# barlettacarmen/CrCNN

Measured on NVIDIA B200. Metric: encrypted MNIST images/sec, higher is better.
Workload: dtype u64

## Files before the change

### crcnn_b200/csrc/engine.cu

```cuda
#include <cuda_runtime.h>
#include <dlfcn.h>
#include <algorithm>
#include <cstdlib>
#include <cstring>
#include <map>
#include <unordered_map>
#include <string>
#include <vector>

#include "../../include/crcnn_b200.h"
#include "kernels.cuh"
#include "params.h"
#include "tc_mac.cuh"
#include "tcn_mac.cuh"
#include "relin32.cuh"
#include "reenc.cuh"

using namespace crcnn;

namespace {

enum KernelClass {
    KC_NTT_FWD = 0, KC_NTT_INV, KC_MAC, KC_PLAIN_EXPAND, KC_POOL, KC_BN, KC_PLAIN_OP,
    KC_BEHZ_LIFT, KC_SQ_TENSOR, KC_BEHZ_FLOOR, KC_RELIN, KC_PROBE, KC_TC_SPLIT, KC_TC_MAC, KC_TCN_SPLIT, KC_TCN_MAC, KC_RELIN32, KC_REENC, KC_COUNT
};
const char *kClassNames[KC_COUNT] = {"ntt_forward", "ntt_inverse", "weighted_sum_mac", "plain_expand_ntt", "pool_sum",
                                     "batch_norm", "plain_op", "behz_lift", "square_tensor", "behz_floor_sk",
                                     "relinearize", "imad_probe", "tc_plane_split", "weighted_sum_tc_i8", "tcn_plane_split",
                                     "weighted_sum_tcn_i8", "relinearize_u32", "reencrypt"};

thread_local std::string g_create_error;

}

struct crcnn_tensor {
    long count;
    int size;
    int ntt;
    uint64_t *d;
};

static long next_plain_serial() { static long s = 0; return ++s; }

struct crcnn_plain {
    long serial = next_plain_serial();
    long count;
    bool sparse_shape = false;
    std::vector<uint32_t> off, idx;
    std::vector<uint64_t> val;
    uint32_t *d_off = nullptr, *d_idx = nullptr;
    uint64_t *d_val = nullptr;
    uint64_t *ntt_mul = nullptr;
    uint64_t *ntt_mul_sh = nullptr;
    uint64_t *ntt_add = nullptr;
    uint64_t *coef_add = nullptr;
    int tap_state = 0;
    int tc_state = 0;
    int8_t *tc_A = nullptr;
    int tc_R = 0, tc_Kpad = 0;
    uint8_t *tcn_W = nullptr;
    int tcn_R = 0;
    bool tcn_pre = false;
    uint64_t *fused_C = nullptr, *fused_Csh = nullptr, *fused_D = nullptr;
    long fused_scale = 0, fused_mean = 0;
    int add_mult = 1;
    bool dense_only = false;
    crcnn_plain *folded_w = nullptr, *folded_b = nullptr;
    long folded_key[9] = {0, 0, 0, 0, 0, 0, 0, 0, 0};
};

struct crcnn_evk {
    uint64_t *d = nullptr;
    long key_off[MAXK];
    int digits[MAXK];
    int dbc;
    bool has_r32 = false;
    Relin32 r32;
};

struct crcnn_keys {
    uint64_t *sk = nullptr;
    uint64_t *pk = nullptr;
    ReencConsts c;
    BudgetConsts b;
};

struct crcnn_ctx {
    int device = 0;
    cudaStream_t stream = nullptr;
    HostParams hp;
    DeviceParams *dP = nullptr;
    std::vector<void *> owned;
    int n = 0, logn = 0, K = 0, S = 0;
    int chunk_terms = 1 << 30;
    size_t weight_cache_bytes = 24ull << 30;
    int sm_count = 148;
    int tc_mode = 1;
    int tc_min_fanin = 256;
    int tc_min_outputs = 32;
    int tap_mode = 1;
    int relin_mode = 1;
    int tcn_mode = 1;
    int sq_lean = 1;
    int tcn_preshift = 1;
    int tcn_fold = 1;
    size_t tc_scratch_bytes = 12ull << 30;
    std::string err;
    std::map<std::vector<int>, int *> index_cache;
    std::unordered_map<void *, size_t> big_size;
    std::multimap<size_t, void *> big_free;
    size_t big_cached = 0, big_cache_cap = 64ull << 30;
    long long st_big_malloc = 0, st_big_hit = 0, st_big_bypass = 0, st_flush = 0, st_small_malloc = 0;
    uint64_t *stage = nullptr;
    size_t stage_bytes = 0;
    bool prof_on = false;
    long launches[KC_COUNT] = {0};
    double ms[KC_COUNT] = {0};
    double work_bytes[KC_COUNT] = {0};
    double work_ops[KC_COUNT] = {0};
    struct Pending { int cls; cudaEvent_t a, b; };
    std::vector<Pending> pending;
    std::vector<cudaEvent_t> event_pool;
};

namespace {

int fail(crcnn_ctx *ctx, int code, const std::string &msg) {
    if (ctx) ctx->err = msg; else g_create_error = msg;
    return code;
}

#define CU(call)                                                                                       \
    do {                                                                                               \
        cudaError_t e__ = (call);                                                                      \
        if (e__ != cudaSuccess) {                                                                      \
            int code__ = (e__ == cudaErrorMemoryAllocation) ? CRCNN_ERR_OUT_OF_MEMORY : CRCNN_ERR_CUDA; \
            return fail(ctx, code__, std::string(#call) + ": " + cudaGetErrorString(e__));            \
        }                                                                                              \
    } while (0)

#define REQUIRE(cond, msg) \
    do { if (!(cond)) return fail(ctx, CRCNN_ERR_INVALID_ARGUMENT, msg); } while (0)

struct ProfScope {
    crcnn_ctx *c; int cls; cudaEvent_t a = nullptr, b = nullptr;
    ProfScope(crcnn_ctx *ctx, int k, double bytes = 0, double ops = 0) : c(ctx), cls(k) {
        c->launches[cls]++;
        c->work_bytes[cls] += bytes;
        c->work_ops[cls] += ops;
        if (!c->prof_on) return;
        auto get = [&]() { cudaEvent_t e; if (!c->event_pool.empty()) { e = c->event_pool.back(); c->event_pool.pop_back(); } else cudaEventCreate(&e); return e; };
        a = get(); b = get();
        cudaEventRecord(a, c->stream);
    }
    ~ProfScope() {
        if (!a) return;
        cudaEventRecord(b, c->stream);
        c->pending.push_back({cls, a, b});
    }
};

void prof_collect(crcnn_ctx *c) {
    for (auto &p : c->pending) {
        cudaEventSynchronize(p.b);
        float t = 0;
        cudaEventElapsedTime(&t, p.a, p.b);
        c->ms[p.cls] += t;
        c->event_pool.push_back(p.a);
        c->event_pool.push_back(p.b);
    }
    c->pending.clear();
}

inline size_t poly_words(const crcnn_ctx *c) { return (size_t)c->K * c->n; }
inline double lp_bytes(const crcnn_ctx *c, double polys) { return polys * c->n * 8.0; }
inline double lp_bfly(const crcnn_ctx *c, double polys) { return polys * (c->n / 2) * c->logn; }

constexpr size_t kBigBlock = 32ull << 20;
void big_cache_flush(crcnn_ctx *ctx) {
    for (auto &kv : ctx->big_free) { ctx->big_size.erase(kv.second); cudaFreeAsync(kv.second, ctx->stream); }
    ctx->big_free.clear();
    ctx->big_cached = 0;
}
int dev_alloc(crcnn_ctx *ctx, size_t bytes, void **out) {
    *out = nullptr;
    if (bytes == 0) return CRCNN_OK;
    if (bytes >= kBigBlock) {
        auto it = ctx->big_free.find(bytes);
        if (it != ctx->big_free.end()) {
            *out = it->second;
            ctx->big_cached -= bytes;
            ctx->big_free.erase(it);
            ctx->st_big_hit++;
            return CRCNN_OK;
        }
        ctx->st_big_malloc++;
    } else {
        ctx->st_small_malloc++;
    }
    cudaError_t e = cudaMallocAsync(out, bytes, ctx->stream);
    if (e == cudaErrorMemoryAllocation && !ctx->big_free.empty()) {
        cudaGetLastError();
        ctx->st_flush++;
        big_cache_flush(ctx);
        e = cudaMallocAsync(out, bytes, ctx->stream);
    }
    CU(e);
    if (bytes >= kBigBlock) ctx->big_size[*out] = bytes;
    return CRCNN_OK;
}
void dev_free(crcnn_ctx *ctx, void *p) {
    if (!p) return;
    auto it = ctx->big_size.find(p);
    if (it != ctx->big_size.end()) {
        if (ctx->big_cached + it->second <= ctx->big_cache_cap) {
            ctx->big_free.insert({it->second, p});
            ctx->big_cached += it->second;
            return;
        }
        ctx->big_size.erase(it);
        ctx->st_big_bypass++;
    }
    cudaFreeAsync(p, ctx->stream);
}

int new_tensor(crcnn_ctx *ctx, long count, int size, int ntt, crcnn_tensor **out) {
    auto *t = new crcnn_tensor{count, size, ntt, nullptr};
    int rc = dev_alloc(ctx, (size_t)count * size * poly_words(ctx) * 8, (void **)&t->d);
    if (rc) { delete t; return rc; }
    *out = t;
    return CRCNN_OK;
}

int ntt_inplace(crcnn_ctx *ctx, uint64_t *d, long npolys, int slot_base, int slot_count, bool inverse) {
    ProfScope ps(ctx, inverse ? KC_NTT_INV : KC_NTT_FWD, 2 * lp_bytes(ctx, npolys), lp_bfly(ctx, npolys));
    CU(launch_ntt(ctx->dP, ctx->logn, d, npolys, slot_base, slot_count, inverse, ctx->stream));
    return CRCNN_OK;
}

int ensure_domain(crcnn_ctx *ctx, crcnn_tensor *t, int want_ntt) {
    if (t->ntt == want_ntt) return CRCNN_OK;
    int rc = ntt_inplace(ctx, t->d, t->count * t->size * ctx->K, 0, ctx->K, !want_ntt);
    if (rc) return rc;
    t->ntt = want_ntt;
    return CRCNN_OK;
}

enum PlainForm { PF_NTT_MUL, PF_NTT_ADD, PF_COEF_ADD };

int expand_range(crcnn_ctx *ctx, crcnn_plain *p, long first, long count, PlainForm f, uint64_t *dst) {
    ProfScope ps(ctx, KC_PLAIN_EXPAND, lp_bytes(ctx, (double)count * ctx->K), f != PF_COEF_ADD ? lp_bfly(ctx, (double)count * ctx->K) : 0);
    CU(launch_plain_expand(ctx->dP, ctx->logn, ctx->K, p->d_off, p->d_idx, p->d_val, first, count,
                           (f == PF_NTT_MUL ? 0 : 1) | (p->sparse_shape ? 2 : 0), f != PF_COEF_ADD, dst, ctx->stream));
    return CRCNN_OK;
}

// ... 195 lines not shown
    dev_free(ctx, w->ntt_mul); w->ntt_mul = nullptr;
    if (w->ntt_mul_sh) { dev_free(ctx, w->ntt_mul_sh); w->ntt_mul_sh = nullptr; }
    w->tcn_R = R;
    w->tcn_pre = preshift;
    return CRCNN_OK;
}

int run_weighted_sum_tcn(crcnn_ctx *ctx, crcnn_tensor *in, crcnn_plain *w, crcnn_plain *b, const int *d_index, int R,
                         int Npos, int Pimg, int m_first, int M, crcnn_tensor *out) {
    const int Kpad = tcn_kpad(R), ncols = 2 * Npos, total = ctx->K * ctx->n;
    const int variant = ctx->tcn_mode >= 2 ? ctx->tcn_mode - 1 : 0;
    const bool want_pre = ctx->tcn_preshift && tcn_preshift_shape(R, ncols, M, variant) &&
                          7 * tcn_w_bytes(7, (int)(w->count / R), Kpad, ctx->K, ctx->n) <= ctx->weight_cache_bytes;
    int rc = ensure_domain(ctx, in, 1);
    if (!rc) rc = ensure_form(ctx, b, PF_NTT_ADD);
    if (!rc) rc = ensure_tcn_weights(ctx, w, R, want_pre);
    if (rc) return rc;
    const size_t pw = poly_words(ctx);
    const size_t per_slot = tcn_x_bytes_per_slot(7, ncols, Kpad);
    long chunk = (long)(ctx->tc_scratch_bytes / per_slot) / 32 * 32;
    chunk = std::max<long>(32, std::min<long>(chunk, total));
    uint8_t *scratch = nullptr;
    rc = dev_alloc(ctx, (size_t)chunk * per_slot, (void **)&scratch);
    if (rc) return rc;
    TcnSplitArgs s{};
    s.src = in->d; s.index = d_index; s.dst = scratch; s.item_polys = 2;
    s.R = R; s.Kpad = Kpad; s.planes = 7; s.ncols = ncols; s.n = ctx->n; s.K = ctx->K;
    TcnMacArgs a{};
    a.W = w->tcn_W; a.X = scratch; a.bias = b->ntt_add + (size_t)m_first * pw; a.out = out->d;
    a.Mall = (int)(w->count / R); a.m_first = m_first; a.M = M;
    a.R = R; a.Kpad = Kpad; a.planes = 7; a.ncols = ncols;
    a.Pimg = Pimg; a.Mtotal = M; a.m0 = 0; a.n = ctx->n; a.K = ctx->K;
    a.variant = variant;
    a.preshift = want_pre && w->tcn_pre;
    a.use_fold = ctx->tcn_fold;
    for (int j = 0; j < ctx->K; j++) a.fold[j] = tcn_fold_make(ctx->hp.d.tab[j].mod.q);
    for (long s0 = 0; s0 < total && !rc; s0 += chunk) {
        const int ns = (int)std::min<long>(chunk, total - s0);
        s.slot0 = a.slot0 = (int)s0; s.nslots = a.nslots = ns;
        const double xbytes = (double)ns * per_slot;
        cudaError_t e;
        { ProfScope ps(ctx, KC_TCN_SPLIT, (double)ncols * R * ns * 8.0 + xbytes, 0); e = launch_tcn_split(s, ctx->stream); }
        if (e == cudaSuccess) {
            ProfScope ps(ctx, KC_TCN_MAC, xbytes + (double)ns * 7 * M * Kpad * (a.preshift ? 7 : 1) + (double)ncols * M * ns * 8.0, (double)ns * ncols * M * R * 49.0);
            e = launch_tcn_mac(ctx->dP, a, ctx->sm_count, ctx->stream);
        }
        if (e != cudaSuccess) rc = fail(ctx, CRCNN_ERR_CUDA, std::string("limb-split tensor-core weighted sum: ") + cudaGetErrorString(e));
    }
    dev_free(ctx, scratch);
    if (!rc) out->ntt = 1;
    return rc;
}

int run_weighted_sum(crcnn_ctx *ctx, crcnn_tensor *in, crcnn_plain *w, crcnn_plain *b, const int *d_index, int R,
                     int Npos, int Pimg, int Mall, int m_first, int M, crcnn_tensor *out) {
    if (ctx->tc_mode && R >= ctx->tc_min_fanin && (ctx->tc_mode == 2 || Mall >= ctx->tc_min_outputs) && w->sparse_shape && tc_mac_available() == cudaSuccess) {
        int rc = ensure_tc_form(ctx, w, R);
        if (rc) return rc;
        if (w->tc_state == 1) return run_weighted_sum_tc(ctx, in, w, b, d_index, R, Npos, Pimg, m_first, M, out);
    }
    if (ctx->tcn_mode && tcn_planes_for(ctx->hp.d) == 7 && R <= TCN_MAX_R && w->count % R == 0 && tc_mac_available() == cudaSuccess &&
        (w->tcn_W || tcn_w_bytes(7, (int)(w->count / R), tcn_kpad(R), ctx->K, ctx->n) <= ctx->weight_cache_bytes))
        return run_weighted_sum_tcn(ctx, in, w, b, d_index, R, Npos, Pimg, m_first, M, out);
    int rc = ensure_domain(ctx, in, 1);
    if (rc) return rc;
    rc = ensure_form(ctx, b, PF_NTT_ADD);
    if (rc) return rc;
    MacArgs a{};
    a.x = in->d; a.in_index = d_index; a.out = out->d;
    a.R = R; a.Npos = Npos; a.Pimg = Pimg; a.Mtotal = M; a.K = ctx->K; a.n = ctx->n;
    a.chunk_terms = ctx->chunk_terms;
    const size_t pw = poly_words(ctx);
    const size_t all_bytes = (size_t)w->count * pw * 8;
    if (w->ntt_mul || all_bytes <= ctx->weight_cache_bytes) {
        rc = ensure_form(ctx, w, PF_NTT_MUL);
        if (rc) return rc;
        a.w = w->ntt_mul + (size_t)m_first * R * pw;
        a.bias = b->ntt_add + (size_t)m_first * pw;
        a.M = M; a.m0 = 0;
        ProfScope ps(ctx, KC_MAC, lp_bytes(ctx, ((double)in->count + (double)M * Npos) * 2 * ctx->K + (double)M * R * ctx->K),
                     (double)M * Npos * R * 2 * ctx->K * ctx->n);
        CU(launch_mac(ctx->dP, a, ctx->stream));
        return CRCNN_OK;
    }
    long rows = (long)std::max<size_t>(1, ctx->weight_cache_bytes / ((size_t)R * pw * 8));
    rows = std::min<long>(rows, M);
    uint64_t *scratch = nullptr;
    rc = dev_alloc(ctx, (size_t)rows * R * pw * 8, (void **)&scratch);
    if (rc) return rc;
    for (long m0 = 0; m0 < M; m0 += rows) {
        long cur = std::min<long>(rows, M - m0);
        rc = expand_range(ctx, w, (long)(m_first + m0) * R, cur * R, PF_NTT_MUL, scratch);
        if (rc) break;
        a.w = scratch; a.bias = b->ntt_add + (size_t)(m_first + m0) * pw;
        a.M = (int)cur; a.m0 = (int)m0;
        ProfScope ps(ctx, KC_MAC, lp_bytes(ctx, ((double)in->count + (double)cur * Npos) * 2 * ctx->K + (double)cur * R * ctx->K),
                     (double)cur * Npos * R * 2 * ctx->K * ctx->n);
        cudaError_t e = launch_mac(ctx->dP, a, ctx->stream);
        if (e != cudaSuccess) { rc = fail(ctx, CRCNN_ERR_CUDA, cudaGetErrorString(e)); break; }
    }
    dev_free(ctx, scratch);
    return rc;
}

int upload_rows(crcnn_ctx *ctx, const uint64_t *host, size_t rows, uint64_t *dst, cudaStream_t s) {
    const size_t n = ctx->n;
    if (rows * n * 8 < (8u << 20)) {
        CU(cudaMemcpy2DAsync(dst, n * 8, host, (n + 1) * 8, n * 8, rows, cudaMemcpyHostToDevice, s));
        return CRCNN_OK;
    }
    uint64_t *stage = nullptr;
    CU(cudaMallocAsync((void **)&stage, rows * (n + 1) * 8, s));
    cudaError_t e = cudaMemcpyAsync(stage, host, rows * (n + 1) * 8, cudaMemcpyHostToDevice, s);
    if (e == cudaSuccess) e = launch_strip_pad(stage, dst, (long)rows, (int)n, s);
    cudaFreeAsync(stage, s);
    if (e != cudaSuccess) return fail(ctx, CRCNN_ERR_CUDA, std::string("upload: ") + cudaGetErrorString(e));
    return CRCNN_OK;
}

}

extern "C" {

const char *crcnn_last_error(const crcnn_ctx *ctx) { return ctx ? ctx->err.c_str() : g_create_error.c_str(); }

int crcnn_ctx_create(int n, int K, const uint64_t *q, uint64_t t, int device, crcnn_ctx **out) {
    crcnn_ctx *ctx = nullptr;
    if (!out || !q) return fail(nullptr, CRCNN_ERR_INVALID_ARGUMENT, "null argument");
    *out = nullptr;
    int ndev = 0;
    if (cudaGetDeviceCount(&ndev) != cudaSuccess || ndev == 0)
        return fail(nullptr, CRCNN_ERR_NO_DEVICE, "no CUDA device: crcnn_b200 has no CPU fallback");
    if (device < 0 || device >= ndev) return fail(nullptr, CRCNN_ERR_INVALID_ARGUMENT, "bad device ordinal");
    HostParams hp;
    try {
        hp = derive_params(n, K, q, t);
    } catch (const std::exception &e) {
        return fail(nullptr, CRCNN_ERR_INVALID_ARGUMENT, e.what());
    }
    CU(cudaSetDevice(device));
    auto *c = new crcnn_ctx();
    c->device = device; c->n = n; c->K = K; c->S = hp.d.S; c->logn = hp.d.logn;
    int maxbits = 0;
    for (int i = 0; i < K; i++) { int b = 0; for (uint64_t v = q[i]; v; v >>= 1) b++; maxbits = std::max(maxbits, b); }
    int spare = 128 - 2 * maxbits;
    c->chunk_terms = spare >= 30 ? (1 << 30) : (1 << spare);
    cudaDeviceGetAttribute(&c->sm_count, cudaDevAttrMultiProcessorCount, device);
    if (const char *e = getenv("CRCNN_TC")) c->tc_mode = atoi(e);
    if (const char *e = getenv("CRCNN_TCN")) c->tcn_mode = atoi(e);
    if (const char *e = getenv("CRCNN_TAP")) c->tap_mode = atoi(e);
    if (const char *e = getenv("CRCNN_TCN_FOLD")) c->tcn_fold = atoi(e);
    if (const char *e = getenv("CRCNN_TCN2_PRESHIFT")) c->tcn_preshift = atoi(e);
    if (const char *e = getenv("CRCNN_SQ_LEAN")) c->sq_lean = atoi(e);
    cudaMemPool_t pool;
    if (cudaDeviceGetDefaultMemPool(&pool, device) == cudaSuccess) {
        uint64_t thr = UINT64_MAX;
        cudaMemPoolSetAttribute(pool, cudaMemPoolAttrReleaseThreshold, &thr);
    }
    {
        size_t fr = 0, tot = 0;
        if (cudaMemGetInfo(&fr, &tot) == cudaSuccess && tot) c->big_cache_cap = tot / 4 * 3;
    }
    int slots = K + hp.d.S;
    auto up = [&](const std::vector<uint64_t> &v, const uint64_t **dst) -> cudaError_t {
        void *d = nullptr;
        cudaError_t e = cudaMalloc(&d, v.size() * 8);
        if (e != cudaSuccess) return e;
        c->owned.push_back(d);
        *dst = (const uint64_t *)d;
        return cudaMemcpy(d, v.data(), v.size() * 8, cudaMemcpyHostToDevice);
    };
    cudaError_t e = cudaSuccess;
    for (int s = 0; s < slots && e == cudaSuccess; s++) {
        std::vector<uint64_t> fw(2 * (size_t)n), bw(2 * (size_t)n);
        for (int i = 0; i < n; i++) {
            fw[2 * i] = hp.w[s][i]; fw[2 * i + 1] = hp.wp[s][i];
            bw[2 * i] = hp.iwf[s][i]; bw[2 * i + 1] = hp.iwfp[s][i];
        }
        e = up(fw, &hp.d.tab[s].w);
        if (e == cudaSuccess) e = up(bw, &hp.d.tab[s].iw);
        const int NG = n >> 4;
        std::vector<uint64_t> fl(2 * (size_t)16 * NG, 0), bl(2 * (size_t)16 * NG, 0);
        for (int G = 0; G < NG; G++)
            for (int st = 0; st < 4; st++) {
                for (int lb = 0; lb < (1 << st); lb++) {
                    const size_t at = 2 * ((size_t)((1 << st) - 1 + lb) * NG + G), from = 2 * ((((size_t)NG + G) << st) + lb);
                    fl[at] = fw[from]; fl[at + 1] = fw[from + 1];
                }
                for (int lb = 0; lb < (1 << (3 - st)); lb++) {
                    const size_t at = 2 * ((size_t)(16 - (16 >> st) + lb) * NG + G);
                    const size_t from = 2 * ((size_t)((n >> 1) >> st) + ((size_t)G << (3 - st)) + lb);
                    bl[at] = bw[from]; bl[at + 1] = bw[from + 1];
                }
            }
        if (e == cudaSuccess) e = up(fl, &hp.d.tab[s].wl);
        if (e == cudaSuccess) e = up(bl, &hp.d.tab[s].iwl);
        hp.d.tab[s].tf = nullptr;
        if (e == cudaSuccess && s < K) e = up(hp.tf[s], &hp.d.tab[s].tf);
    }
    if (e == cudaSuccess) e = cudaMalloc((void **)&c->dP, sizeof(DeviceParams));
    if (e == cudaSuccess) e = cudaMemcpy(c->dP, &hp.d, sizeof(DeviceParams), cudaMemcpyHostToDevice);
    if (e != cudaSuccess) {
        std::string m = cudaGetErrorString(e);
        for (void *p : c->owned) cudaFree(p);
        if (c->dP) cudaFree(c->dP);
        delete c;
        return fail(nullptr, CRCNN_ERR_CUDA, "context setup: " + m);
    }
    c->hp = std::move(hp);
    *out = c;
    return CRCNN_OK;
}

int crcnn_ctx_destroy(crcnn_ctx *ctx) {
    if (!ctx) return CRCNN_OK;
    cudaSetDevice(ctx->device);
    big_cache_flush(ctx);
    cudaStreamSynchronize(ctx->stream);
    prof_collect(ctx);
    for (auto e : ctx->event_pool) cudaEventDestroy(e);
    for (auto &kv : ctx->index_cache) cudaFree(kv.second);
    if (ctx->stage) cudaFree(ctx->stage);
    for (void *p : ctx->owned) cudaFree(p);
    cudaFree(ctx->dP);
    delete ctx;
    return CRCNN_OK;
}

int crcnn_ctx_set_stream(crcnn_ctx *ctx, void *cuda_stream) {
    if (!ctx) return CRCNN_ERR_INVALID_ARGUMENT;
    CU(cudaStreamSynchronize(ctx->stream));
    ctx->stream = (cudaStream_t)cuda_stream;
    return CRCNN_OK;
}

int crcnn_ctx_sync(crcnn_ctx *ctx) {
    if (!ctx) return CRCNN_ERR_INVALID_ARGUMENT;
    CU(cudaStreamSynchronize(ctx->stream));
    prof_collect(ctx);
    return CRCNN_OK;
}

int crcnn_ctx_alloc_stats(crcnn_ctx *ctx, long long out[6]) {
    if (!ctx || !out) return CRCNN_ERR_INVALID_ARGUMENT;
    out[0] = ctx->st_big_malloc; out[1] = ctx->st_big_hit; out[2] = ctx->st_big_bypass; out[3] = ctx->st_flush;
    out[4] = ctx->st_small_malloc; out[5] = (long long)ctx->big_cached;
    return CRCNN_OK;
}

int crcnn_ctx_set_weight_cache_bytes(crcnn_ctx *ctx, size_t bytes) {
    if (!ctx) return CRCNN_ERR_INVALID_ARGUMENT;
    ctx->weight_cache_bytes = bytes;
    return CRCNN_OK;
}

int crcnn_ctx_set_tensor_core_mode(crcnn_ctx *ctx, int mode, int min_fanin, size_t scratch_bytes) {
    if (!ctx) return CRCNN_ERR_INVALID_ARGUMENT;
    REQUIRE(mode >= 0 && mode <= 2, "tensor-core mode must be 0, 1 or 2");
    ctx->tc_mode = mode;
    if (min_fanin > 0) ctx->tc_min_fanin = min_fanin;
    if (scratch_bytes > 0) ctx->tc_scratch_bytes = scratch_bytes;
    return CRCNN_OK;
}

int crcnn_ctx_set_limb_split_mode(crcnn_ctx *ctx, int mode) {
    if (!ctx) return CRCNN_ERR_INVALID_ARGUMENT;
    REQUIRE(mode >= 0 && mode <= 3, "limb-split mode must be 0 (off), 1 (on), 2 (row-major kernel) or 3 (column-major kernel)");
    ctx->tcn_mode = mode;
    return CRCNN_OK;
}

int crcnn_ctx_set_limb_split_reduction(crcnn_ctx *ctx, int mode) {
    if (!ctx) return CRCNN_ERR_INVALID_ARGUMENT;
    REQUIRE(mode == 0 || mode == 1, "limb-split reduction must be 0 (128-bit recombination + Barrett) or 1 (folded through 2^k - delta)");
    ctx->tcn_fold = mode;
    return CRCNN_OK;
}

int crcnn_ctx_set_relin_mode(crcnn_ctx *ctx, int mode) {
    if (!ctx) return CRCNN_ERR_INVALID_ARGUMENT;
    REQUIRE(mode == 0 || mode == 1, "relinearize mode must be 0 (64-bit transforms) or 1 (word-size auxiliary primes)");
    ctx->relin_mode = mode;
    return CRCNN_OK;
}

int crcnn_ctx_ntt_table(const crcnn_ctx *ctx_c, int slot, int which, uint64_t *out) {
    crcnn_ctx *ctx = const_cast<crcnn_ctx *>(ctx_c);
    if (!ctx) return CRCNN_ERR_INVALID_ARGUMENT;
    REQUIRE(out && slot >= 0 && slot < ctx->K + ctx->S && which >= 0 && which < 4, "bad table selector");
    const auto &v = which == 0 ? ctx->hp.w[slot] : which == 1 ? ctx->hp.wp[slot] : which == 2 ? ctx->hp.iw[slot] : ctx->hp.iwp[slot];
    memcpy(out, v.data(), v.size() * 8);
    return CRCNN_OK;
}

int crcnn_ctx_bsk_count(const crcnn_ctx *ctx) { return ctx ? ctx->S : CRCNN_ERR_INVALID_ARGUMENT; }

int crcnn_tensor_upload_ex(crcnn_ctx *ctx, const uint64_t *host, long count, int size, int ntt_form, crcnn_tensor **out) {
    if (!ctx) return CRCNN_ERR_INVALID_ARGUMENT;
    REQUIRE(host && out && count >= 0 && size >= 2 && size <= 3, "bad tensor upload arguments");
    CU(cudaSetDevice(ctx->device));
    crcnn_tensor *t = nullptr;
    int rc = new_tensor(ctx, count, size, ntt_form ? 1 : 0, &t);
    if (rc) return rc;
    const size_t n = ctx->n, rows = (size_t)count * size * ctx->K;
    if (rows) {
        int rc2 = upload_rows(ctx, host, rows, t->d, ctx->stream);
// ... 594 lines not shown
        int rc = get_index_table(ctx, key, table, &d_index);
        if (rc) return rc;
    } else {
        d_index = ctx->index_cache[key];
    }
    int rc = ensure_pool_bn_consts(ctx, scale, mean, invstd);
    if (rc) return rc;
    crcnn_tensor *o = nullptr;
    rc = new_tensor(ctx, Nout, 2, 1, &o);
    if (rc) return rc;
    {
        ProfScope ps(ctx, KC_POOL, lp_bytes(ctx, ((double)in->count + Nout) * 2 * ctx->K), (double)Nout * (R + 1) * 2 * ctx->K * ctx->n);
        cudaError_t e = launch_pool(ctx->dP, ctx->n, ctx->K, in->d, d_index, Nout, R, invstd->fused_C, invstd->fused_Csh, true, o->d, ctx->stream,
                                    xo * yo, zd, invstd->fused_D);
        if (e != cudaSuccess) { crcnn_tensor_free(ctx, o); return fail(ctx, CRCNN_ERR_CUDA, cudaGetErrorString(e)); }
    }
    *out = o;
    return CRCNN_OK;
}

int crcnn_conv_pool_bn_forward_shard(crcnn_ctx *ctx, crcnn_tensor *in, crcnn_plain *w, crcnn_plain *b, int batch, int xd, int yd, int zd,
                                     int xs, int ys, int xf, int yf, int nf, int pxs, int pys, int pxf, int pyf, crcnn_plain *scale,
                                     crcnn_plain *mean, crcnn_plain *invstd, int k0, int kc, crcnn_tensor **out) {
    if (!ctx) return CRCNN_ERR_INVALID_ARGUMENT;
    REQUIRE(k0 >= 0 && kc >= 0 && k0 + kc <= nf, "bad output-channel shard");
    REQUIRE(in && w && b && mean && invstd && out, "null argument");
    REQUIRE(batch > 0 && xd > 0 && yd > 0 && zd > 0 && xs > 0 && ys > 0 && xf > 0 && yf > 0 && nf > 0 && xf <= xd && yf <= yd,
            "bad convolution geometry");
    const int cxo = (xd - xf) / xs + 1, cyo = (yd - yf) / ys + 1;
    REQUIRE(pxs > 0 && pys > 0 && pxf > 0 && pyf > 0 && pxf <= cxo && pyf <= cyo, "bad pooling geometry");
    const int pxo = (cxo - pxf) / pxs + 1, pyo = (cyo - pyf) / pys + 1;
    const int Rp = pxf * pyf, R = zd * xf * yf;
    REQUIRE(in->size == 2 && in->count == (long)batch * zd * xd * yd, "input tensor does not match the layer geometry");
    REQUIRE(w->count == (long)nf * R && b->count == nf, "kernel/bias count does not match the layer geometry");
    REQUIRE((!scale || scale->count >= 1) && mean->count == nf && invstd->count == nf, "mean/var count does not match the channel count");
    CU(cudaSetDevice(ctx->device));
    const bool pooled_grid = pxs <= pxf && pys <= pyf && xs <= xf && ys <= yf && pxs * xs <= xf && pys * ys <= yf && Rp <= 64 && sum_fits_64(ctx, Rp) &&
                             ctx->tcn_mode && tcn_planes_for(ctx->hp.d) == 7 && R <= TCN_MAX_R && tc_mac_available() == cudaSuccess &&
                             tcn_w_bytes(7, nf, tcn_kpad(R), ctx->K, ctx->n) <= ctx->weight_cache_bytes && !getenv("CRCNN_NO_POOLED_CONV");
    if (!pooled_grid) {
        if (k0 != 0 || kc != nf)
            return fail(ctx, CRCNN_ERR_UNSUPPORTED, "channel shards of conv + pool + batch-norm need the pooled-grid path");
        crcnn_tensor *mid = nullptr;
        int rc = crcnn_conv_forward(ctx, in, w, b, batch, xd, yd, zd, xs, ys, xf, yf, nf, &mid);
        if (rc) return rc;
        rc = crcnn_pool_bn_forward(ctx, mid, batch, cxo, cyo, nf, pxs, pys, pxf, pyf, scale, mean, invstd, out);
        crcnn_tensor_free(ctx, mid);
        return rc;
    }
    int rc = ensure_pool_bn_consts(ctx, scale, mean, invstd);
    if (rc) return rc;
    const long key[9] = {b->serial, scale ? scale->serial : -1, mean->serial, invstd->serial, (long)Rp, 0, 0, 0, 0};
    if (!w->folded_w || memcmp(key, w->folded_key, sizeof(key)) != 0) {
        if (w->folded_w) { crcnn_plain_free(ctx, w->folded_w); w->folded_w = nullptr; }
        if (w->folded_b) { crcnn_plain_free(ctx, w->folded_b); w->folded_b = nullptr; }
        const size_t pw = poly_words(ctx);
        rc = make_plain(ctx, std::vector<uint32_t>(w->off), std::vector<uint32_t>(w->idx), std::vector<uint64_t>(w->val), &w->folded_w);
        if (rc) return rc;
        w->folded_w->sparse_shape = false;
        w->folded_w->tc_state = -1; w->folded_w->tap_state = -1;
        rc = ensure_form(ctx, w->folded_w, PF_NTT_MUL);
        if (rc) return rc;
        CU(launch_fold_affine(ctx->dP, w->folded_w->ntt_mul, (long)nf * R, (long)pw, R, invstd->fused_C, nullptr, ctx->stream));
        rc = make_plain(ctx, std::vector<uint32_t>(b->off), std::vector<uint32_t>(b->idx), std::vector<uint64_t>(b->val), &w->folded_b);
        if (rc) return rc;
        w->folded_b->add_mult = Rp;
        rc = ensure_form(ctx, w->folded_b, PF_NTT_ADD);
        if (rc) return rc;
        CU(launch_fold_affine(ctx->dP, w->folded_b->ntt_add, (long)nf, (long)pw, 1, invstd->fused_C, invstd->fused_D, ctx->stream));
        memcpy(w->folded_key, key, sizeof(key));
    }
    const int sxd = xd - (pxf - 1) * xs, syd = yd - (pyf - 1) * ys;
    const int Nsum = batch * zd * sxd * syd;
    std::vector<int> skey = {4, batch, xd, yd, zd, xs, ys, pxf, pyf};
    const int *d_index = nullptr;
    if (ctx->index_cache.find(skey) == ctx->index_cache.end()) {
        std::vector<int> table((size_t)Nsum * Rp);
        size_t o = 0;
        for (int bz = 0; bz < batch * zd; bz++)
            for (int u = 0; u < sxd; u++)
                for (int v = 0; v < syd; v++)
                    for (int a = 0; a < pxf; a++)
                        for (int c = 0; c < pyf; c++) table[o++] = (bz * xd + u + a * xs) * yd + v + c * ys;
        rc = get_index_table(ctx, skey, table, &d_index);
        if (rc) return rc;
    } else {
        d_index = ctx->index_cache[skey];
    }
    crcnn_tensor *sums = nullptr, *pooled = nullptr;
    rc = new_tensor(ctx, Nsum, 2, in->ntt, &sums);
    if (rc) return rc;
    {
        ProfScope ps(ctx, KC_POOL, lp_bytes(ctx, ((double)in->count + Nsum) * 2 * ctx->K), (double)Nsum * Rp * 2 * ctx->K * ctx->n);
        cudaError_t e = launch_pool(ctx->dP, ctx->n, ctx->K, in->d, d_index, Nsum, Rp, nullptr, nullptr, true, sums->d, ctx->stream);
        if (e != cudaSuccess) { crcnn_tensor_free(ctx, sums); return fail(ctx, CRCNN_ERR_CUDA, cudaGetErrorString(e)); }
    }
    rc = crcnn_conv_forward_shard(ctx, sums, w->folded_w, w->folded_b, batch, sxd, syd, zd, pxs * xs, pys * ys, xf, yf, nf, k0, kc, &pooled);
    crcnn_tensor_free(ctx, sums);
    if (rc) return rc;
    if (pooled->count != (long)batch * kc * pxo * pyo || !pooled->ntt) {
        crcnn_tensor_free(ctx, pooled);
        return fail(ctx, CRCNN_ERR_UNSUPPORTED, "pooled-grid convolution produced an unexpected shape");
    }
    *out = pooled;
    return CRCNN_OK;
}

int crcnn_conv_pool_bn_forward(crcnn_ctx *ctx, crcnn_tensor *in, crcnn_plain *w, crcnn_plain *b, int batch, int xd, int yd, int zd,
                               int xs, int ys, int xf, int yf, int nf, int pxs, int pys, int pxf, int pyf, crcnn_plain *scale,
                               crcnn_plain *mean, crcnn_plain *invstd, crcnn_tensor **out) {
    return crcnn_conv_pool_bn_forward_shard(ctx, in, w, b, batch, xd, yd, zd, xs, ys, xf, yf, nf, pxs, pys, pxf, pyf, scale, mean, invstd, 0, nf, out);
}

int crcnn_bn_forward(crcnn_ctx *ctx, crcnn_tensor *in, int batch, int zd, int xd, int yd, crcnn_plain *mean,
                     crcnn_plain *invstd, crcnn_tensor **out) {
    if (!ctx) return CRCNN_ERR_INVALID_ARGUMENT;
    REQUIRE(in && mean && invstd && out, "null argument");
    REQUIRE(batch > 0 && zd > 0 && xd > 0 && yd > 0, "bad batch-norm geometry");
    REQUIRE(in->size == 2 && in->count == (long)batch * zd * xd * yd, "input tensor does not match the layer geometry");
    REQUIRE(mean->count == zd && invstd->count == zd, "mean/var count does not match the channel count");
    CU(cudaSetDevice(ctx->device));
    if (!in->ntt && ctx->tap_mode && tap_eligible(ctx, invstd)) {
        int rc = ensure_form(ctx, mean, PF_COEF_ADD);
        if (rc) return rc;
        crcnn_tensor *o = nullptr;
        rc = new_tensor(ctx, in->count, 2, 0, &o);
        if (rc) return rc;
        TapMulArgs a{};
        a.in = in->d; a.in_index = nullptr; a.R = 1; a.sub = mean->coef_add;
        a.t_off = invstd->d_off; a.t_idx = invstd->d_idx; a.t_val = invstd->d_val; a.per_channel = xd * yd; a.channels = zd;
        a.out = o->d; a.nout = in->count;
        ProfScope ps(ctx, KC_BN, lp_bytes(ctx, (double)in->count * 4 * ctx->K), (double)in->count * 2 * ctx->K * ctx->n);
        cudaError_t e = launch_tapmul(ctx->dP, ctx->n, ctx->K, a, ctx->stream);
        if (e != cudaSuccess) { crcnn_tensor_free(ctx, o); return fail(ctx, CRCNN_ERR_CUDA, cudaGetErrorString(e)); }
        *out = o;
        return CRCNN_OK;
    }
    int rc = ensure_domain(ctx, in, 1);
    if (!rc) rc = ensure_form(ctx, mean, PF_NTT_ADD);
    if (!rc) rc = ensure_shoup(ctx, invstd);
    if (rc) return rc;
    crcnn_tensor *o = nullptr;
    rc = new_tensor(ctx, in->count, 2, 1, &o);
    if (rc) return rc;
    {
        ProfScope ps(ctx, KC_BN, lp_bytes(ctx, (double)in->count * 4 * ctx->K), (double)in->count * 2 * ctx->K * ctx->n);
        cudaError_t e = launch_bn(ctx->dP, ctx->n, ctx->K, in->d, in->count, xd * yd, zd, mean->ntt_add, invstd->ntt_mul, invstd->ntt_mul_sh, o->d, ctx->stream);
        if (e != cudaSuccess) { crcnn_tensor_free(ctx, o); return fail(ctx, CRCNN_ERR_CUDA, cudaGetErrorString(e)); }
    }
    *out = o;
    return CRCNN_OK;
}

int crcnn_square(crcnn_ctx *ctx, crcnn_tensor *in, crcnn_tensor **out3) {
    if (!ctx) return CRCNN_ERR_INVALID_ARGUMENT;
    REQUIRE(in && out3, "null argument");
    REQUIRE(in->size == 2, "square expects size-2 ciphertexts");
    CU(cudaSetDevice(ctx->device));
    const bool have_ntt = in->ntt != 0;
    const bool lean = ctx->sq_lean != 0, fold = lean && behz_fold_ok(ctx->hp.d), copy_ninv = !(lean && have_ntt);
    crcnn_tensor *o = nullptr;
    int rc = new_tensor(ctx, in->count, 3, 0, &o);
    if (rc) return rc;
    const int KS = ctx->K + ctx->S;
    const size_t n = ctx->n, pw = poly_words(ctx);
    const long step = std::max<long>(1, std::min<long>(in->count, (long)((2ull << 30) / (5 * (size_t)KS * n * 8))));
    uint64_t *ext = nullptr, *prod = nullptr, *coef = nullptr;
    rc = dev_alloc(ctx, (size_t)step * 2 * KS * n * 8, (void **)&ext);
    if (!rc) rc = dev_alloc(ctx, (size_t)step * 3 * KS * n * 8, (void **)&prod);
    if (!rc && have_ntt) rc = dev_alloc(ctx, (size_t)step * 2 * pw * 8, (void **)&coef);
    if (rc) { crcnn_tensor_free(ctx, o); return rc; }
    for (long c0 = 0; c0 < in->count && !rc; c0 += step) {
        const long cur = std::min<long>(step, in->count - c0);
        const uint64_t *src = in->d + c0 * 2 * pw;
        cudaError_t e = cudaSuccess;
        if (have_ntt) {
            ProfScope ps(ctx, KC_NTT_INV, 2 * lp_bytes(ctx, (double)cur * 2 * ctx->K), lp_bfly(ctx, (double)cur * 2 * ctx->K));
            e = launch_ntt_grouped(ctx->dP, ctx->logn, coef, cur * 2 * ctx->K, 0, ctx->K, true, ctx->K, 0, ctx->stream, src,
                                   nullptr, 1, 1, copy_ninv);
        }
        if (e == cudaSuccess) { ProfScope ps(ctx, KC_BEHZ_LIFT, lp_bytes(ctx, (double)cur * 2 * (ctx->K + (have_ntt ? ctx->S : KS))), (double)cur * 2 * n * ctx->S * (ctx->K + 1)); e = launch_behz_lift(ctx->hp.d, ctx->n, have_ntt ? coef : src, have_ntt ? src : nullptr, cur, ext, ctx->stream, copy_ninv); }
        if (e == cudaSuccess) {
            if (have_ntt) {
                ProfScope ps(ctx, KC_NTT_FWD, 2 * lp_bytes(ctx, (double)cur * 2 * ctx->S), lp_bfly(ctx, (double)cur * 2 * ctx->S));
                e = launch_ntt_grouped(ctx->dP, ctx->logn, ext, cur * 2 * ctx->S, ctx->K, ctx->S, false, KS, ctx->K, ctx->stream);
            } else {
                ProfScope ps(ctx, KC_NTT_FWD, 2 * lp_bytes(ctx, (double)cur * 2 * KS), lp_bfly(ctx, (double)cur * 2 * KS));
                e = launch_ntt(ctx->dP, ctx->logn, ext, cur * 2 * KS, 0, KS, false, ctx->stream);
            }
        }
        if (e == cudaSuccess) {
            ProfScope ps(ctx, KC_SQ_TENSOR, lp_bytes(ctx, (double)cur * 5 * KS), lp_bfly(ctx, (double)cur * 3 * KS));
            e = launch_ntt_inv_tensor(ctx->dP, ctx->logn, ext, have_ntt ? src : nullptr, cur, KS, prod, fold, !lean, ctx->stream);
        }
        if (e == cudaSuccess) { ProfScope ps(ctx, KC_BEHZ_FLOOR, lp_bytes(ctx, (double)cur * 3 * (KS + ctx->K)),
                                                     (double)cur * 3 * n * (ctx->S * (ctx->K + 1) + ctx->S + ctx->K * ctx->S)); e = launch_behz_floor(ctx->hp.d, ctx->n, prod, cur, o->d + c0 * 3 * pw, ctx->stream, !lean); }
        if (e != cudaSuccess) rc = fail(ctx, CRCNN_ERR_CUDA, cudaGetErrorString(e));
    }
    dev_free(ctx, coef);
    dev_free(ctx, ext); dev_free(ctx, prod);
    if (rc) { crcnn_tensor_free(ctx, o); return rc; }
    *out3 = o;
    return CRCNN_OK;
}

int crcnn_relinearize(crcnn_ctx *ctx, crcnn_tensor *in3, crcnn_evk *evk, crcnn_tensor **out2) {
    if (!ctx) return CRCNN_ERR_INVALID_ARGUMENT;
    REQUIRE(in3 && evk && out2, "null argument");
    REQUIRE(in3->size == 3, "relinearize expects size-3 ciphertexts");
    int total_digits = 0;
    for (int i = 0; i < ctx->K; i++) {
        int bits = 0; for (uint64_t v = ctx->hp.d.tab[i].mod.q; v; v >>= 1) bits++;
        REQUIRE(evk->digits[i] * evk->dbc >= bits, "not enough evaluation keys");
        total_digits += evk->digits[i];
    }
    REQUIRE(total_digits <= 63, "too many key digits for 128-bit lazy accumulation");
    CU(cudaSetDevice(ctx->device));
    int rc = ensure_domain(ctx, in3, 0);
    if (rc) return rc;
    crcnn_tensor *o = nullptr;
    rc = new_tensor(ctx, in3->count, 2, 0, &o);
    if (rc) return rc;
    const size_t pw = poly_words(ctx);
    if (evk->has_r32 && ctx->relin_mode == 1) {
        const Relin32Consts &c = evk->r32.c;
        const size_t per_ct = relin32_scratch_bytes(ctx->n, ctx->K, c);
        const long step = std::max<long>(1, std::min<long>(std::min<long>(in3->count, 200000), (long)((2ull << 30) / per_ct)));
        void *scratch = nullptr;
        rc = dev_alloc(ctx, (size_t)step * per_ct, &scratch);
        if (rc) { crcnn_tensor_free(ctx, o); return rc; }
        for (long c0 = 0; c0 < in3->count && !rc; c0 += step) {
            const long cnt = std::min<long>(step, in3->count - c0);
            ProfScope ps(ctx, KC_RELIN32, lp_bytes(ctx, (double)cnt * 5 * ctx->K),
                         lp_bfly(ctx, (double)cnt * (c.D + 2 * ctx->K) * c.S3));
            cudaError_t e = relin32_run(ctx->dP, ctx->logn, ctx->K, evk->r32, in3->d + c0 * 3 * pw, o->d + c0 * 2 * pw, cnt, scratch, ctx->stream);
            if (e != cudaSuccess) rc = fail(ctx, CRCNN_ERR_CUDA, cudaGetErrorString(e));
        }
        dev_free(ctx, scratch);
        if (rc) { crcnn_tensor_free(ctx, o); return rc; }
        *out2 = o;
        return CRCNN_OK;
    }
    RelinArgs a{};
    a.evk = evk->d; a.dbc = evk->dbc;
    for (int i = 0; i < MAXK; i++) { a.key_off[i] = evk->key_off[i]; a.digits[i] = evk->digits[i]; }
    const size_t per_ct = (size_t)(1 + total_digits + 2) * pw * 8;
    const long step = std::max<long>(1, std::min<long>(in3->count, (long)((2ull << 30) / per_ct)));
    uint64_t *scratch = nullptr;
    rc = dev_alloc(ctx, (size_t)step * per_ct, (void **)&scratch);
    if (rc) { crcnn_tensor_free(ctx, o); return rc; }
    a.dsc = scratch;
    a.dig = scratch + (size_t)step * pw;
    a.acc = a.dig + (size_t)step * total_digits * pw;
    for (long c0 = 0; c0 < in3->count && !rc; c0 += step) {
        a.count = std::min<long>(step, in3->count - c0);
        a.in3 = in3->d + c0 * 3 * pw;
        a.out = o->d + c0 * 2 * pw;
        cudaError_t e;
        { ProfScope ps(ctx, KC_RELIN, lp_bytes(ctx, (double)a.count * 3 * ctx->K), lp_bfly(ctx, (double)a.count * total_digits * ctx->K)); e = launch_relin(ctx->dP, ctx->logn, ctx->K, a, ctx->stream); }
        if (e == cudaSuccess) {
            ProfScope ps(ctx, KC_NTT_INV, 2 * lp_bytes(ctx, (double)a.count * 2 * ctx->K) + lp_bytes(ctx, (double)a.count * 2 * ctx->K), lp_bfly(ctx, (double)a.count * 2 * ctx->K));
            e = launch_ntt_grouped(ctx->dP, ctx->logn, a.out, a.count * 2 * ctx->K, 0, ctx->K, true, ctx->K, 0, ctx->stream, a.acc, a.in3,
                                   2 * ctx->K, 3 * ctx->K);
        }
        if (e != cudaSuccess) rc = fail(ctx, CRCNN_ERR_CUDA, cudaGetErrorString(e));
    }
    dev_free(ctx, scratch);
    if (rc) { crcnn_tensor_free(ctx, o); return rc; }
    *out2 = o;
    return CRCNN_OK;
}

int crcnn_square_forward(crcnn_ctx *ctx, crcnn_tensor *in, crcnn_evk *evk, crcnn_tensor **out) {
    if (!ctx) return CRCNN_ERR_INVALID_ARGUMENT;
    crcnn_tensor *t3 = nullptr;
    int rc = crcnn_square(ctx, in, &t3);
    if (rc) return rc;
    rc = crcnn_relinearize(ctx, t3, evk, out);
    crcnn_tensor_free(ctx, t3);
    return rc;
}

int crcnn_transform_to_ntt(crcnn_ctx *ctx, crcnn_tensor *t) {
    if (!ctx) return CRCNN_ERR_INVALID_ARGUMENT;
    REQUIRE(t, "null argument");
    REQUIRE(!t->ntt, "tensor is already in NTT form");
    CU(cudaSetDevice(ctx->device));
    return ensure_domain(ctx, t, 1);
}
int crcnn_transform_from_ntt(crcnn_ctx *ctx, crcnn_tensor *t) {
    if (!ctx) return CRCNN_ERR_INVALID_ARGUMENT;
    REQUIRE(t, "null argument");
    REQUIRE(t->ntt, "tensor is not in NTT form");
    CU(cudaSetDevice(ctx->device));
    return ensure_domain(ctx, t, 0);
}

int crcnn_plain_op(crcnn_ctx *ctx, crcnn_tensor *t, crcnn_plain *p, long index, int op) {
    if (!ctx) return CRCNN_ERR_INVALID_ARGUMENT;
    REQUIRE(t && p && index >= 0 && index < p->count && op >= 0 && op <= 2, "bad plain_op arguments");
    CU(cudaSetDevice(ctx->device));
    int rc;
    const uint64_t *pl, *pl_sh = nullptr;
    if (op == 0) {
        rc = ensure_domain(ctx, t, 1);
        if (!rc) rc = ensure_shoup(ctx, p);
        if (rc) return rc;
        pl = p->ntt_mul + index * poly_words(ctx);
        pl_sh = p->ntt_mul_sh + index * poly_words(ctx);
    } else {
        rc = ensure_form(ctx, p, t->ntt ? PF_NTT_ADD : PF_COEF_ADD);
        if (rc) return rc;
        pl = (t->ntt ? p->ntt_add : p->coef_add) + index * poly_words(ctx);
    }
    ProfScope ps(ctx, KC_PLAIN_OP, lp_bytes(ctx, (double)t->count * (op == 0 ? t->size : 1) * 2 * ctx->K), (double)t->count * (op == 0 ? t->size : 1) * ctx->K * ctx->n);
    CU(launch_plain_op(ctx->dP, ctx->n, ctx->K, t->d, t->count, t->size, pl, pl_sh, op, ctx->stream));
    return CRCNN_OK;
}

int crcnn_add_many(crcnn_ctx *ctx, crcnn_tensor *t, crcnn_tensor **out) {
    if (!ctx) return CRCNN_ERR_INVALID_ARGUMENT;
    REQUIRE(t && out, "null argument");
    REQUIRE(t->count >= 1, "encrypteds cannot be empty");
    REQUIRE(t->size == 2, "add_many is implemented for size-2 ciphertexts");
    CU(cudaSetDevice(ctx->device));
    auto pass = [&](const uint64_t *src, long first, int nout, int g, uint64_t *dst) -> int {
        std::vector<int> key = {4, (int)first, nout, g};
        const int *d_index = nullptr;
        auto it = ctx->index_cache.find(key);
        if (it == ctx->index_cache.end()) {
            std::vector<int> table((size_t)nout * g);
            for (size_t i = 0; i < table.size(); i++) table[i] = (int)(first + (long)i);
            int rc = get_index_table(ctx, key, table, &d_index);
            if (rc) return rc;
        } else d_index = it->second;
        ProfScope ps(ctx, KC_POOL, lp_bytes(ctx, ((double)nout * g + nout) * 2 * ctx->K), (double)nout * g * 2 * ctx->K * ctx->n);
        CU(launch_pool(ctx->dP, ctx->n, ctx->K, src, d_index, nout, g, nullptr, nullptr, sum_fits_64(ctx, g), dst, ctx->stream));
        return CRCNN_OK;
    };
    crcnn_tensor *o = nullptr;
    int rc = new_tensor(ctx, 1, 2, t->ntt, &o);
    if (rc) return rc;
    if (t->count <= 128) {
        rc = pass(t->d, 0, 1, (int)t->count, o->d);
    } else {
        int g = 1;
        while ((long)g * g < t->count) g++;
        const long full = t->count / g, tail = t->count % g, groups = full + (tail ? 1 : 0);
        crcnn_tensor *part = nullptr;
        rc = new_tensor(ctx, groups, 2, t->ntt, &part);
        if (!rc) rc = pass(t->d, 0, (int)full, g, part->d);
        if (!rc && tail) rc = pass(t->d, full * g, 1, (int)tail, part->d + full * 2 * poly_words(ctx));
        if (!rc) rc = pass(part->d, 0, 1, (int)groups, o->d);
        crcnn_tensor_free(ctx, part);
    }
    if (rc) { crcnn_tensor_free(ctx, o); return rc; }
    *out = o;
    return CRCNN_OK;
}

int crcnn_prof_enable(crcnn_ctx *ctx, int on) {
    if (!ctx) return CRCNN_ERR_INVALID_ARGUMENT;
    ctx->prof_on = on != 0;
    return CRCNN_OK;
}
int crcnn_prof_reset(crcnn_ctx *ctx) {
    if (!ctx) return CRCNN_ERR_INVALID_ARGUMENT;
    prof_collect(ctx);
    for (int i = 0; i < KC_COUNT; i++) { ctx->launches[i] = 0; ctx->ms[i] = 0; ctx->work_bytes[i] = 0; ctx->work_ops[i] = 0; }
    return CRCNN_OK;
}
int crcnn_prof_count(crcnn_ctx *ctx) { return ctx ? (int)KC_COUNT : (int)CRCNN_ERR_INVALID_ARGUMENT; }
int crcnn_prof_get(crcnn_ctx *ctx, int cls, char *name, long *launches, double *ms) {
    if (!ctx) return CRCNN_ERR_INVALID_ARGUMENT;
    REQUIRE(cls >= 0 && cls < KC_COUNT, "bad kernel class");
    prof_collect(ctx);
    if (name) { strncpy(name, kClassNames[cls], 31); name[31] = 0; }
    if (launches) *launches = ctx->launches[cls];
    if (ms) *ms = ctx->ms[cls];
    return CRCNN_OK;
}

int crcnn_prof_get_work(crcnn_ctx *ctx, int cls, double *bytes, double *ops) {
    if (!ctx) return CRCNN_ERR_INVALID_ARGUMENT;
    REQUIRE(cls >= 0 && cls < KC_COUNT, "bad kernel class");
    if (bytes) *bytes = ctx->work_bytes[cls];
    if (ops) *ops = ctx->work_ops[cls];
    return CRCNN_OK;
}

int crcnn_probe_pipe(crcnn_ctx *ctx, int which, int blocks, int threads, int iters, double *ms, double *ops) {
    if (!ctx) return CRCNN_ERR_INVALID_ARGUMENT;
    REQUIRE(which >= 0 && which <= 4 && blocks > 0 && threads > 0 && threads <= 1024 && iters > 0 && ms, "bad probe arguments");
    CU(cudaSetDevice(ctx->device));
    uint64_t *sink = nullptr;
    int rc = dev_alloc(ctx, 8, (void **)&sink);
    if (rc) return rc;
    cudaEvent_t a, b;
    CU(cudaEventCreate(&a));
    CU(cudaEventCreate(&b));
    ctx->launches[KC_PROBE]++;
    double work = 0;
    CU(cudaEventRecord(a, ctx->stream));
    if (which == 0) { CU(launch_imad_probe(blocks, threads, iters, sink, ctx->stream)); work = (double)blocks * threads * iters * 8.0; }
    else if (which == 1) { CU(launch_imad_wide_probe(blocks, threads, iters, sink, ctx->stream)); work = (double)blocks * threads * iters * 16.0; }
    else CU(launch_umma_i8_probe(blocks, iters, which - 2, &work, ctx->stream));
    CU(cudaEventRecord(b, ctx->stream));
    CU(cudaEventSynchronize(b));
    float t = 0;
    cudaEventElapsedTime(&t, a, b);
    *ms = t;
    if (ops) *ops = work;
    cudaEventDestroy(a); cudaEventDestroy(b);
    dev_free(ctx, sink);
    return CRCNN_OK;
}
int crcnn_probe_imad(crcnn_ctx *ctx, int blocks, int threads, int iters, double *ms) {
    return crcnn_probe_pipe(ctx, 0, blocks, threads, iters, ms, nullptr);
}

int crcnn_pinned_alloc(size_t bytes, void **out) {
    if (!out) return CRCNN_ERR_INVALID_ARGUMENT;
    *out = nullptr;
    cudaError_t e = cudaHostAlloc(out, bytes, cudaHostAllocDefault);
    if (e != cudaSuccess) { g_create_error = std::string("cudaHostAlloc: ") + cudaGetErrorString(e); return e == cudaErrorMemoryAllocation ? CRCNN_ERR_OUT_OF_MEMORY : CRCNN_ERR_CUDA; }
    return CRCNN_OK;
}
int crcnn_pinned_free(void *p) { return (!p || cudaFreeHost(p) == cudaSuccess) ? CRCNN_OK : CRCNN_ERR_CUDA; }

int crcnn_stream_create(crcnn_ctx *ctx, void **stream) {
    if (!ctx) return CRCNN_ERR_INVALID_ARGUMENT;
    REQUIRE(stream, "null argument");
    CU(cudaSetDevice(ctx->device));
// ... 363 lines not shown
```

### crcnn_b200/csrc/host_selftest.cpp

```cpp
#include <cinttypes>
#include <cstdio>
#include <cstdlib>
#include <vector>
#include "params.h"

using namespace crcnn;

static uint64_t fnv(const std::vector<uint64_t> &v) {
    uint64_t h = 1469598103934665603ULL;
    for (uint64_t x : v) { h ^= x; h *= 1099511628211ULL; }
    return h;
}

int main(int argc, char **argv) {
    if (argc < 4) { fprintf(stderr, "usage: host_selftest n t q...\n"); return 2; }
    int n = atoi(argv[1]);
    uint64_t t = strtoull(argv[2], nullptr, 0);
    std::vector<uint64_t> q;
    for (int i = 3; i < argc; i++) q.push_back(strtoull(argv[i], nullptr, 0));
    try {
        HostParams hp = derive_params(n, (int)q.size(), q.data(), t);
        const DeviceParams &d = hp.d;
        printf("K %d L %d S %d half %" PRIu64 "\n", d.K, d.L, d.S, d.half);
        for (int s = 0; s < d.K + d.S; s++) {
            printf("slot %d q %" PRIu64 " r0 %" PRIu64 " r1 %" PRIu64 " root %" PRIu64 " w %" PRIu64 " wp %" PRIu64 " iw %" PRIu64 " iwp %" PRIu64 "\n",
                   s, d.tab[s].mod.q, d.tab[s].mod.r0, d.tab[s].mod.r1, hp.roots[s], fnv(hp.w[s]), fnv(hp.wp[s]), fnv(hp.iw[s]), fnv(hp.iwp[s]));
        }
        for (int j = 0; j < d.K; j++)
            printf("prime %d delta %" PRIu64 " rho %" PRIu64 " lift %" PRIu64 "\n", j, d.delta[j], d.rho[j], d.lift_inc[j]);
        uint64_t x = 0x123456789abcdef1ULL, y = 0xfedcba9876543211ULL;
        for (int s = 0; s < d.K + d.S; s++) {
            const Mod &m = d.tab[s].mod;
            for (int it = 0; it < 1000; it++) {
                x = x * 6364136223846793005ULL + 1442695040888963407ULL;
                y = y * 2862933555777941757ULL + 3037000493ULL;
                uint64_t a = x % (4 * m.q), b = y % m.q;
                uint64_t want = (uint64_t)(((unsigned __int128)a * b) % m.q);
                if (mulmod(a, b, m) != want) { printf("MULMOD MISMATCH\n"); return 1; }
                uint64_t wp = (uint64_t)((((unsigned __int128)b) << 64) / m.q);
                uint64_t lazy = mulshoup_lazy(a, b, wp, m.q);
                if (lazy >= 2 * m.q || lazy % m.q != want) { printf("SHOUP MISMATCH\n"); return 1; }
            }
        }
        for (int j = 0; j < d.K; j++) {
            const Mod &m = d.tab[j].mod;
            const TcnFold f = tcn_fold_make(m.q);
            printf("fold %d ok %u T %u delta %u\n", j, f.ok, f.T, f.delta);
            if (!f.ok) continue;
            for (int it = 0; it < 200000; it++) {
                uint32_t s[13];
                const int mode = it % 8;
                for (int w = 0; w < 13; w++) {
                    x = x * 6364136223846793005ULL + 1442695040888963407ULL;
                    const uint32_t r = (uint32_t)(x >> 33);
                    s[w] = mode == 0 ? 0x7fffffffu : mode == 1 ? 0u : mode == 2 ? ((x >> 20) & 1 ? 0x7fffffffu : 0u)
                         : mode == 3 ? 7u * 4096u * 255u * 255u - (r & 3) : mode == 4 ? (r >> (x & 31)) : r;
                }
                y = y * 2862933555777941757ULL + 3037000493ULL;
                const uint64_t bias = mode == 0 ? m.q - 1 : (it & 1) ? y % m.q : 0;
                unsigned __int128 z = 0;
                for (int w = 12; w >= 0; w--) z = (z << 8) + s[w];
                const uint64_t want = (uint64_t)((z + bias) % m.q);
                if (tcn_fold_reduce(s, bias, f, m.q) != want) { printf("FOLD MISMATCH\n"); return 1; }
            }
        }
        for (int j = 0; j < d.K; j++) {
            const Mod &m = d.tab[j].mod;
            const TcnFold f = tcn_fold_make(m.q);
            long checked = 0;
            for (int it = 0; it < 20000; it++) {
                x = x * 6364136223846793005ULL + 1442695040888963407ULL;
                y = y * 2862933555777941757ULL + 3037000493ULL;
                const uint64_t W = it < 2 ? m.q - 1 : x % m.q, X = it < 2 ? m.q - 1 : y % m.q;
                uint32_t C[7] = {0, 0, 0, 0, 0, 0, 0};
                for (int b = 0; b < 7; b++) {
                    const uint64_t wb = (uint64_t)(((unsigned __int128)1 << (8 * b)) % m.q);
                    const uint64_t wbp = (uint64_t)(((unsigned __int128)wb << 64) / m.q);
                    uint64_t Wb = mulshoup_lazy(W, wb, wbp, m.q);
                    Wb = Wb >= m.q ? Wb - m.q : Wb;
                    if (Wb != (uint64_t)(((unsigned __int128)W << (8 * b)) % m.q)) { printf("PRESHIFT MISMATCH\n"); return 1; }
                    uint64_t back = 0;
                    for (int a = 6; a >= 0; a--) back = (back << 8) | ((Wb >> (8 * a)) & 0xff);
                    if (back != Wb) { printf("PLANE MISMATCH\n"); return 1; }
                    for (int a = 0; a < 7; a++) C[a] += (uint32_t)(((X >> (8 * b)) & 0xff) * ((Wb >> (8 * a)) & 0xff));
                }
                const uint64_t bias = (it & 1) ? y % m.q : 0;
                const uint64_t want = (uint64_t)(((unsigned __int128)W * X + bias) % m.q);
                const U128 z = tcn7_combine(C);
                if (addmod(barrett128(z, m), bias, m.q) != want) { printf("SEVEN-CLASS MISMATCH\n"); return 1; }
                if (f.ok7 && tcn7_fold_reduce(C, bias, f, m.q) != want) { printf("FOLD7 MISMATCH\n"); return 1; }
                checked++;
            }
            const uint32_t cmax = 7u * 4096u * 255u * 255u;
            for (int it = 0; it < 2000 && f.ok7; it++) {
                uint32_t C[7];
                x = x * 6364136223846793005ULL + 1442695040888963407ULL;
                for (int a = 0; a < 7; a++) C[a] = it == 0 ? cmax : cmax - (uint32_t)((x >> (4 * a)) % 4096);
                const uint64_t bias = it == 0 ? m.q - 1 : x % m.q;
                unsigned __int128 z = 0;
                for (int a = 6; a >= 0; a--) z = (z << 8) + C[a];
                if (z >> 80) { printf("FOLD7 BOUND\n"); return 1; }
                if (tcn7_fold_reduce(C, bias, f, m.q) != (uint64_t)((z + bias) % m.q)) { printf("FOLD7 MISMATCH\n"); return 1; }
                checked++;
            }
            printf("fold7 %d ok7 %u checked %ld\n", j, f.ok7, checked);
        }
        for (int sidx = 0; sidx < d.K + d.S; sidx++) {
            const Mod &m = d.tab[sidx].mod;
            const Fold128 f = fold128_make(m.q);
            printf("fold128 %d ok %u delta %u\n", sidx, f.ok, f.delta);
            if (!f.ok) continue;
            for (int it = 0; it < 200000; it++) {
                x = x * 6364136223846793005ULL + 1442695040888963407ULL;
                y = y * 2862933555777941757ULL + 3037000493ULL;
                U128 z;
                const int mode = it % 8;
                z.lo = mode == 0 ? ~0ull : mode == 1 ? 0 : mode == 2 ? m.q - 1 : mode == 3 ? m.q : x;
                z.hi = mode == 0 ? ~0ull : mode == 1 ? 0 : mode == 2 ? 0 : mode == 3 ? (y >> (y & 63)) : mode == 4 ? (y >> 40) : y;
                const uint64_t want = (uint64_t)(((((unsigned __int128)z.hi) << 64) | z.lo) % m.q);
                if (reduce128_fold(z, f) != want || barrett128(z, m) != want) { printf("FOLD128 MISMATCH\n"); return 1; }
            }
        }
        typedef unsigned __int128 u128;
        for (int s = 0; s < d.K + d.S; s++) {
            const uint64_t q = d.tab[s].mod.q;
            const bool ok_ninv = (u128)d.tab[s].ninv * (uint64_t)n % q == 1;
            bool ok = ok_ninv;
            if (s < d.K) {
                ok = ok && d.mt_inv_qhat_n[s] < q && (u128)d.mt_inv_qhat_n[s] * (uint64_t)n % q == d.mt_inv_qhat[s];
                ok = ok && d.fl_c_n[s] < q && (u128)d.fl_c_n[s] * (uint64_t)n % q == d.fl_c[s];
            } else {
                ok = ok && d.fl_T_n[s - d.K] < q && (u128)d.fl_T_n[s - d.K] * (uint64_t)n % q == d.fl_T[s - d.K];
            }
            printf("ninv %d ok %d\n", s, ok ? 1 : 0);
            if (!ok) { printf("NINV CONSTANT MISMATCH\n"); return 1; }
        }
        for (int s = 0; s < d.K + d.S; s++) {
            const uint64_t q = d.tab[s].mod.q, nq = 0 - q;
            const uint64_t ws[] = {0, 1, q - 1, q / 2, 0x5555555555555555ULL % q, 0};
            long checked = 0;
            for (int wi = 0; wi < 6; wi++) {
                uint64_t w = ws[wi];
                for (int it = 0; it < 20000; it++) {
                    x = x * 6364136223846793005ULL + 1442695040888963407ULL;
                    y = y * 2862933555777941757ULL + 3037000493ULL;
                    if (wi == 5) w = y % q;
                    const uint64_t wp = (uint64_t)(((u128)w << 64) / q);
                    const int mode = it % 8;
                    const uint64_t yv = mode == 0 ? 0 : mode == 1 ? ~0ull : mode == 2 ? (x % (~0ull / q + 1)) * q
                                      : mode == 3 ? (~0ull / q) * q : mode == 4 ? q - 1 : mode == 5 ? 8 * q - 1 - (x & 7) : x;
                    const uint64_t r = mulshoup_lazy4(yv, w, wp, nq);
                    if (r >= 4 * q || r % q != (uint64_t)((u128)w * yv % q)) { printf("SHOUP4 MISMATCH\n"); return 1; }
                    const uint64_t a = x % q;
                    const U128 z = sqr128(a);
                    if (((u128)z.hi << 64 | z.lo) != (u128)a * a) { printf("SQR128 MISMATCH\n"); return 1; }
                    checked++;
                }
            }
            printf("shoup4 %d checked %ld\n", s, checked);
            const int k = reduce64_shape_k(q);
            if (k) {
                for (int it = 0; it < 200000; it++) {
                    x = x * 6364136223846793005ULL + 1442695040888963407ULL;
                    const int mode = it % 6;
                    const uint64_t v = mode == 0 ? ~0ull : mode == 1 ? 0 : mode == 2 ? q : mode == 3 ? q - 1 : mode == 4 ? (x % 16) * q + (x >> 60) : x;
                    if (reduce64_shape(v, q, k) != v % q || reduce64(v, d.tab[s].mod) != v % q) { printf("REDUCE64 MISMATCH\n"); return 1; }
                }
            }
            printf("reduce64_shape %d k %d\n", s, k);
        }
        for (int i = 4; i >= 0; i--) {
            double vals[] = {0.0867, -3.25, 0.0, 1.0, 2.8215};
            std::vector<uint32_t> idx; std::vector<uint64_t> val;
            encode_fractional_sparse(vals[i], n, t, idx, val);
            printf("enc %.4f nnz %zu", vals[i], idx.size());
            for (size_t e = 0; e < idx.size(); e++) printf(" %u:%" PRIu64, idx[e], val[e]);
            printf("\n");
        }
        printf("OK\n");
    } catch (const std::exception &e) {
        printf("ERROR %s\n", e.what());
        return 1;
    }
    return 0;
}
```

### crcnn_b200/csrc/kernels.cu

```cuda
#include "kernels.cuh"
#include "devcfg.cuh"
#include "ntt.cuh"
#include <cstdlib>
#include <cstring>

namespace crcnn {

template <int LOGN>
__global__ void __launch_bounds__(NttPlan<LOGN>::THREADS, NttPlan<LOGN>::MIN_CTAS)
ntt_fwd_kernel(uint64_t *__restrict__ data, const DeviceParams *__restrict__ P, int slot_base, int slot_count, int group_polys,
               int group_off) {
    extern __shared__ uint64_t sm[];
    const long p = blockIdx.x;
    const NttTable tb = P->tab[slot_base + (int)(p % slot_count)];
    uint64_t *poly = data + ((p / slot_count) * group_polys + group_off + p % slot_count) * (1L << LOGN);
    ntt_forward_to_smem<LOGN>(sm, poly, tb);
    smem_store_poly_canonical<LOGN>(sm, poly, tb.mod);
}

template <int LOGN, bool NINV>
__global__ void __launch_bounds__(NttPlan<LOGN>::THREADS, NttPlan<LOGN>::MIN_CTAS)
ntt_inv_kernel(uint64_t *__restrict__ data, const DeviceParams *__restrict__ P, int slot_base, int slot_count, int group_polys,
               int group_off, const uint64_t *__restrict__ src, const uint64_t *__restrict__ addend, int add_group, int add_stride) {
    extern __shared__ uint64_t sm[];
// ... 586 lines not shown
}

cudaError_t launch_tapmul(const DeviceParams *P, int n, int K, const TapMulArgs &a, cudaStream_t stream) {
    if (a.nout <= 0) return cudaSuccess;
    const long blocks = a.nout * 2 * K * (n / TAP_CT);
    if (n % TAP_CT || blocks > 0x7fffffffL) return cudaErrorInvalidValue;
    tapmul_kernel<<<(unsigned)blocks, 256, 0, stream>>>(P, a);
    return cudaGetLastError();
}

__global__ void __launch_bounds__(256)
shoup_companion_kernel(const DeviceParams *__restrict__ P, const uint64_t *__restrict__ data, long words, uint64_t *__restrict__ out) {
    const long w = (long)blockIdx.x * 256 + threadIdx.x;
    if (w >= words) return;
    const uint64_t q = P->tab[(w / P->n) % P->K].mod.q;
    out[w] = (uint64_t)((((unsigned __int128)__ldg(data + w)) << 64) / q);
}

cudaError_t launch_shoup_companion(const DeviceParams *P, const uint64_t *data, long words, uint64_t *out, cudaStream_t stream) {
    if (words <= 0) return cudaSuccess;
    shoup_companion_kernel<<<(unsigned)((words + 255) / 256), 256, 0, stream>>>(P, data, words, out);
    return cudaGetLastError();
}

__global__ void __launch_bounds__(256)
scale_small_kernel(const DeviceParams *__restrict__ P, uint64_t *__restrict__ data, long words, int times) {
    const long w = (long)blockIdx.x * 256 + threadIdx.x;
    if (w >= words) return;
    const uint64_t q = P->tab[(w / P->n) % P->K].mod.q;
    const uint64_t v = data[w];
    uint64_t acc = 0;
    for (int i = 0; i < times; i++) acc = addmod(acc, v, q);
    data[w] = acc;
}

__global__ void __launch_bounds__(256)
fold_affine_kernel(const DeviceParams *__restrict__ P, uint64_t *__restrict__ data, long rows, int group, const uint64_t *__restrict__ C,
                   const uint64_t *__restrict__ D) {
    const long pw = (long)P->K * P->n;
    const long w = (long)blockIdx.x * 256 + threadIdx.x;
    if (w >= rows * pw) return;
    const long row = w / pw, lw = w - row * pw;
    const Mod mod = P->tab[lw / P->n].mod;
    const long cw = (row / group) * pw + lw;
    uint64_t v = mulmod(data[w], __ldg(C + cw), mod);
    if (D) v = submod(v, __ldg(D + cw), mod.q);
    data[w] = v;
}

cudaError_t launch_fold_affine(const DeviceParams *P, uint64_t *data, long rows, long poly_words, int group, const uint64_t *C,
                               const uint64_t *D, cudaStream_t stream) {
    if (rows <= 0) return cudaSuccess;
    fold_affine_kernel<<<(unsigned)((rows * poly_words + 255) / 256), 256, 0, stream>>>(P, data, rows, group, C, D);
    return cudaGetLastError();
}

__global__ void __launch_bounds__(256)
fold_fc_input_affine_kernel(const DeviceParams *__restrict__ P, uint64_t *__restrict__ W, int out_dim, int in_dim, int per_channel,
                            const uint64_t *__restrict__ C, const uint64_t *__restrict__ D, uint64_t *__restrict__ Bias) {
    const long pw = (long)P->K * P->n;
    const long id = (long)blockIdx.x * 256 + threadIdx.x;
    if (id >= (long)out_dim * pw) return;
    const long k = id / pw, lw = id - k * pw;
    const Mod mod = P->tab[lw / P->n].mod;
    uint64_t acc = Bias[k * pw + lw];
    for (int r = 0; r < in_dim; r++) {
        const long cw = (long)(r / per_channel) * pw + lw;
        uint64_t *wp = W + ((long)k * in_dim + r) * pw + lw;
        const uint64_t w = *wp;
        acc = submod(acc, mulmod(w, __ldg(D + cw), mod), mod.q);
        *wp = mulmod(w, __ldg(C + cw), mod);
    }
    Bias[k * pw + lw] = acc;
}

cudaError_t launch_fold_fc_input_affine(const DeviceParams *P, uint64_t *W, int out_dim, int in_dim, long poly_words, int per_channel,
                                        const uint64_t *C, const uint64_t *D, uint64_t *Bias, cudaStream_t stream) {
    if (out_dim <= 0 || in_dim <= 0) return cudaSuccess;
    fold_fc_input_affine_kernel<<<(unsigned)((out_dim * poly_words + 255) / 256), 256, 0, stream>>>(P, W, out_dim, in_dim, per_channel, C, D, Bias);
    return cudaGetLastError();
}

cudaError_t launch_scale_small(const DeviceParams *P, uint64_t *data, long words, int times, cudaStream_t stream) {
    if (words <= 0) return cudaSuccess;
    scale_small_kernel<<<(unsigned)((words + 255) / 256), 256, 0, stream>>>(P, data, words, times);
    return cudaGetLastError();
}

__global__ void __launch_bounds__(256)
plain_op_kernel(const DeviceParams *__restrict__ P, uint64_t *__restrict__ data, int size, const uint64_t *__restrict__ pl,
                const uint64_t *__restrict__ pl_sh, int op) {
    const int n = P->n, K = P->K;
    const long pw = (long)K * n, ctw = size * pw, active = op == 0 ? ctw : pw;
    const long ct = blockIdx.x;
    const long word = ((long)blockIdx.y * 256 + threadIdx.x) * 4;
    if (word >= active) return;
    const long lw = word % pw;
    const int j = (int)(lw / n);
    const Mod mod = P->tab[j].mod;
    ulonglong2 *x = reinterpret_cast<ulonglong2 *>(data + ct * ctw + word);
    const ulonglong2 *w = reinterpret_cast<const ulonglong2 *>(pl + lw);
    ulonglong2 a = x[0], b = x[1];
    const ulonglong2 wa = __ldg(w), wb = __ldg(w + 1);
    if (op == 0) {
        const ulonglong2 *ws = reinterpret_cast<const ulonglong2 *>(pl_sh + lw);
        const ulonglong2 sa = __ldg(ws), sb = __ldg(ws + 1);
        uint64_t r;
        r = mulshoup_lazy(a.x, wa.x, sa.x, mod.q); a.x = r >= mod.q ? r - mod.q : r;
        r = mulshoup_lazy(a.y, wa.y, sa.y, mod.q); a.y = r >= mod.q ? r - mod.q : r;
        r = mulshoup_lazy(b.x, wb.x, sb.x, mod.q); b.x = r >= mod.q ? r - mod.q : r;
        r = mulshoup_lazy(b.y, wb.y, sb.y, mod.q); b.y = r >= mod.q ? r - mod.q : r;
    }
    else if (op == 1) { a.x = addmod(a.x, wa.x, mod.q); a.y = addmod(a.y, wa.y, mod.q); b.x = addmod(b.x, wb.x, mod.q); b.y = addmod(b.y, wb.y, mod.q); }
    else { a.x = submod(a.x, wa.x, mod.q); a.y = submod(a.y, wa.y, mod.q); b.x = submod(b.x, wb.x, mod.q); b.y = submod(b.y, wb.y, mod.q); }
    x[0] = a; x[1] = b;
}

template <int KT, int ST, bool FOLD>
__global__ void __launch_bounds__(128)
behz_lift_kernel(const __grid_constant__ DeviceParams P, const uint64_t *__restrict__ in, const uint64_t *__restrict__ in_ntt,
                 uint64_t *__restrict__ ext) {
    const int n = P.n, K = KT ? KT : P.K, S = KT ? ST : P.S;
    constexpr int KB = KT ? KT : MAXK, SB = KT ? ST : MAXS;
    const int per = n / 128;
    const long poly = blockIdx.x / per;
    const int c = (blockIdx.x % per) * 128 + threadIdx.x;
    const uint64_t *src = in + poly * K * n + c;
    uint64_t *dst = ext + poly * (K + S) * n + c;
    uint64_t y[KB];
    uint32_t zmt = 0;
#pragma unroll
    for (int i = 0; i < KB; i++) {
        if (i < K) {
            uint64_t x = __ldg(src + (long)i * n);
            if (!in_ntt) dst[(long)i * n] = x;
            y[i] = behz_mulmod<FOLD>(x, P.mt_inv_qhat[i], P.tab[i].mod);
            zmt += (uint32_t)y[i] * (uint32_t)P.qhat_mod_mt[i];
        }
    }
    const uint32_t r = zmt * (uint32_t)P.neg_inv_q_mod_mt;
#pragma unroll
    for (int k = 0; k < SB; k++) {
        if (k < S) {
            Acc7 acc = acc7_zero();
#pragma unroll
            for (int i = 0; i < KB; i++)
                if (i < K) mac7(acc, y[i], P.lift_a[k][i]);
            mac7(acc, (uint64_t)r, P.lift_b[k]);
            dst[(long)(K + k) * n] = behz_reduce<FOLD>(acc7_value(acc), P.tab[K + k].mod);
        }
    }
}

template <int KT, int ST, bool FOLD>
__global__ void __launch_bounds__(128)
behz_floor_kernel(const __grid_constant__ DeviceParams P, const uint64_t *__restrict__ prod, uint64_t *__restrict__ out) {
    const int n = P.n, K = KT ? KT : P.K, S = KT ? ST : P.S, L = S - 1;
    constexpr int KB = KT ? KT : MAXK, SB = KT ? ST : MAXS;
    const int per = n / 128;
    const long poly = blockIdx.x / per;
    const int c = (blockIdx.x % per) * 128 + threadIdx.x;
    const uint64_t *src = prod + poly * (K + S) * n + c;
    uint64_t *dst = out + poly * K * n + c;
    uint64_t u[KB], g[SB];
#pragma unroll
    for (int i = 0; i < KB; i++)
        if (i < K) u[i] = behz_mulmod<FOLD>(__ldg(src + (long)i * n), P.fl_c[i], P.tab[i].mod);
    uint64_t f_sk = 0;
#pragma unroll
    for (int k = 0; k < SB; k++)
        if (k < S) {
            Acc7 acc = acc7_zero();
            mac7(acc, __ldg(src + (long)(K + k) * n), P.fl_T[k]);
#pragma unroll
            for (int i = 0; i < KB; i++)
                if (i < K) mac7(acc, u[i], P.fl_N[k][i]);
            uint64_t v = behz_reduce<FOLD>(acc7_value(acc), P.tab[K + k].mod);
            if (k < L) g[k] = v; else f_sk = v;
        }
    const Mod msk = P.tab[K + L].mod;
    Acc7 acc = acc7_zero();
#pragma unroll
    for (int i = 0; i < SB; i++)
        if (i < L) mac7(acc, g[i], P.fl_P[i]);
    mac7(acc, msk.q - f_sk, P.inv_M_mod_msk);
    const uint64_t alpha = behz_reduce<FOLD>(acc7_value(acc), msk);
    const bool centered_neg = alpha > (msk.q >> 1);
    const uint64_t alpha_mag = centered_neg ? msk.q - alpha : alpha;
#pragma unroll
    for (int j = 0; j < KB; j++)
        if (j < K) {
            Acc7 e = acc7_zero();
#pragma unroll
            for (int i = 0; i < SB; i++)
                if (i < L) mac7(e, g[i], P.Mhat_mod_q[j][i]);
            mac7(e, alpha_mag, centered_neg ? P.M_mod_q[j] : P.neg_M_mod_q[j]);
            dst[(long)j * n] = behz_reduce<FOLD>(acc7_value(e), P.tab[j].mod);
        }
}

__global__ void __launch_bounds__(256)
relin_scale_kernel(const DeviceParams *__restrict__ P, const uint64_t *__restrict__ in3, uint64_t *__restrict__ dsc) {
    const int n = P->n, K = P->K;
    const long pw = (long)K * n;
    const long ct = blockIdx.x;
    const long lw = (long)blockIdx.y * 256 + threadIdx.x;
    const int i = (int)(lw / n);
    dsc[ct * pw + lw] = mulmod(__ldg(in3 + (ct * 3 + 2) * pw + lw), P->inv_qhat[i], P->tab[i].mod);
}

struct DigitMap {
    int D;
    unsigned char prime[32];
    unsigned char shift[32];
};

template <int LOGN>
__global__ void __launch_bounds__(NttPlan<LOGN>::THREADS, NttPlan<LOGN>::MIN_CTAS)
ntt_fwd_digits_kernel(const DeviceParams *__restrict__ P, const uint64_t *__restrict__ dsc, DigitMap map, uint64_t mask,
                      uint64_t *__restrict__ dig) {
    extern __shared__ uint64_t sm[];
    constexpr int N = 1 << LOGN;
    const int K = P->K;
    const long b = blockIdx.x;
    const int j = (int)(b % K);
    const int d = (int)((b / K) % map.D);
    const long ct = b / ((long)K * map.D);
    const NttTable tb = P->tab[j];
    const uint64_t *src = dsc + (ct * K + map.prime[d]) * N;
    const int shift = map.shift[d];
    for (int e = threadIdx.x; e < N; e += blockDim.x) sm[ntt_pad(e)] = (__ldg(src + e) >> shift) & mask;
    __syncthreads();
    ntt_forward_in_smem<LOGN>(sm, tb);
    smem_store_poly_canonical<LOGN>(sm, dig + b * N, tb.mod);
}

__global__ void __launch_bounds__(256)
relin_mac_kernel(const DeviceParams *__restrict__ P, const uint64_t *__restrict__ dig, const uint64_t *__restrict__ evk,
                 RelinArgs a, DigitMap map, uint64_t *__restrict__ acc_out) {
    const int n = P->n, K = P->K;
    const long pw = (long)K * n;
    const long ct = blockIdx.x;
    const long lw = (long)blockIdx.y * 256 + threadIdx.x;
    const int j = (int)(lw / n);
    Acc7 acc0 = acc7_zero(), acc1 = acc7_zero();
    const uint64_t *dp = dig + ct * map.D * pw + lw;
    for (int d = 0; d < map.D; d++) {
        const int i = map.prime[d], k = map.shift[d] / a.dbc;
        const uint64_t *key = evk + a.key_off[i] + (long)(2 * k) * pw + lw;
        const uint64_t dv = __ldg(dp + (long)d * pw);
        mac7(acc0, dv, __ldg(key));
        mac7(acc1, dv, __ldg(key + pw));
    }
    const Mod mod = P->tab[j].mod;
    acc_out[(ct * 2) * pw + lw] = barrett128(acc7_value(acc0), mod);
    acc_out[(ct * 2 + 1) * pw + lw] = barrett128(acc7_value(acc1), mod);
}

__global__ void __launch_bounds__(256)
relin_add_kernel(const DeviceParams *__restrict__ P, const uint64_t *__restrict__ in3, const uint64_t *__restrict__ acc,
                 uint64_t *__restrict__ out) {
    const int n = P->n, K = P->K;
    const long pw = (long)K * n;
    const long ct = blockIdx.x;
    const long w = (long)blockIdx.y * 256 + threadIdx.x;
    const uint64_t q = P->tab[(w % pw) / n].mod.q;
    out[ct * 2 * pw + w] = addmod(__ldg(in3 + ct * 3 * pw + w), __ldg(acc + ct * 2 * pw + w), q);
}

template <int LOGN>
static cudaError_t launch_digits_t(const DeviceParams *P, int K, const uint64_t *dsc, const DigitMap &map, uint64_t mask,
                                   long count, uint64_t *dig, cudaStream_t stream) {
    using Pl = NttPlan<LOGN>;
    size_t smem = Pl::SMEM_WORDS * sizeof(uint64_t);
    auto k = ntt_fwd_digits_kernel<LOGN>;
    static DeviceOnce once;
    if (once.first()) {
        cudaFuncSetAttribute(k, cudaFuncAttributeMaxDynamicSharedMemorySize, (int)smem);
        cudaFuncSetAttribute(k, cudaFuncAttributePreferredSharedMemoryCarveout, cudaSharedmemCarveoutMaxShared);
    }
    k<<<(unsigned)(count * map.D * K), Pl::THREADS, smem, stream>>>(P, dsc, map, mask, dig);
    return cudaGetLastError();
}

cudaError_t launch_relin(const DeviceParams *P, int logn, int K, const RelinArgs &a, cudaStream_t stream) {
    if (a.count <= 0) return cudaSuccess;
    const int n = 1 << logn;
    DigitMap map{};
    for (int i = 0; i < K; i++)
        for (int k = 0; k < a.digits[i]; k++) {
            if (map.D >= 32) return cudaErrorInvalidValue;
            map.prime[map.D] = (unsigned char)i;
            map.shift[map.D] = (unsigned char)(k * a.dbc);
            map.D++;
        }
    const uint64_t mask = (1ULL << a.dbc) - 1;
    dim3 g1((unsigned)a.count, (unsigned)((long)K * n / 256));
    relin_scale_kernel<<<g1, 256, 0, stream>>>(P, a.in3, a.dsc);
    cudaError_t e = cudaGetLastError();
    if (e != cudaSuccess) return e;
    switch (logn) {
        case 10: e = launch_digits_t<10>(P, K, a.dsc, map, mask, a.count, a.dig, stream); break;
        case 11: e = launch_digits_t<11>(P, K, a.dsc, map, mask, a.count, a.dig, stream); break;
        case 12: e = launch_digits_t<12>(P, K, a.dsc, map, mask, a.count, a.dig, stream); break;
        case 13: e = launch_digits_t<13>(P, K, a.dsc, map, mask, a.count, a.dig, stream); break;
        case 14: e = launch_digits_t<14>(P, K, a.dsc, map, mask, a.count, a.dig, stream); break;
        default: return cudaErrorInvalidValue;
    }
    if (e != cudaSuccess) return e;
    relin_mac_kernel<<<g1, 256, 0, stream>>>(P, a.dig, a.evk, a, map, a.acc);
    return cudaGetLastError();
}

cudaError_t launch_relin_finish(const DeviceParams *P, int n, int K, const RelinArgs &a, cudaStream_t stream) {
    if (a.count <= 0) return cudaSuccess;
    dim3 g((unsigned)a.count, (unsigned)(2L * K * n / 256));
    relin_add_kernel<<<g, 256, 0, stream>>>(P, a.in3, a.acc, a.out);
    return cudaGetLastError();
}

static int ew_per(int n) { return n % (512 * 4) == 0 ? 4 : (n % (512 * 2) == 0 ? 2 : 1); }

cudaError_t launch_pool(const DeviceParams *P, int n, int K, const uint64_t *in, const int *in_index, int Nout,
                           int R, const uint64_t *scale_ntt, const uint64_t *scale_shoup, bool sum_fits_64, uint64_t *out,
                           cudaStream_t stream, int per_channel, int channels, const uint64_t *sub) {
    if (Nout <= 0) return cudaSuccess;
    const int per = ew_per(n), chunks = (int)(2L * K * n / (512 * per));
    const unsigned grid = (unsigned)((long)Nout * chunks);
    if (sum_fits_64) pool_kernel<true><<<grid, 256, 0, stream>>>(P, in, in_index, R, scale_ntt, scale_shoup, out, chunks, per, per_channel, channels, sub);
    else pool_kernel<false><<<grid, 256, 0, stream>>>(P, in, in_index, R, scale_ntt, scale_shoup, out, chunks, per, per_channel, channels, sub);
    return cudaGetLastError();
}

__global__ void __launch_bounds__(256)
pool_bn_consts_kernel(const DeviceParams *__restrict__ P, const uint64_t *__restrict__ S, const uint64_t *__restrict__ V,
                      const uint64_t *__restrict__ M, long words, uint64_t *__restrict__ C, uint64_t *__restrict__ D) {
    const long w = (long)blockIdx.x * 256 + threadIdx.x;
    if (w >= words) return;
    const long pw = (long)P->K * P->n, lw = w % pw;
    const Mod mod = P->tab[lw / P->n].mod;
    const uint64_t v = __ldg(V + w);
    C[w] = S ? mulmod(__ldg(S + lw), v, mod) : v;
    D[w] = mulmod(__ldg(M + w), v, mod);
}
cudaError_t launch_pool_bn_consts(const DeviceParams *P, const uint64_t *S, const uint64_t *V, const uint64_t *M, long words,
                                  uint64_t *C, uint64_t *D, cudaStream_t stream) {
    if (words <= 0) return cudaSuccess;
    pool_bn_consts_kernel<<<(unsigned)((words + 255) / 256), 256, 0, stream>>>(P, S, V, M, words, C, D);
    return cudaGetLastError();
}

cudaError_t launch_bn(const DeviceParams *P, int n, int K, const uint64_t *in, long count, int per_channel,
                         int channels, const uint64_t *mean_ntt, const uint64_t *invstd_ntt, const uint64_t *invstd_shoup,
                         uint64_t *out, cudaStream_t stream) {
    if (count <= 0) return cudaSuccess;
    const int per = ew_per(n), chunks = (int)(2L * K * n / (512 * per));
    const unsigned grid = (unsigned)(count * chunks);
    bn_kernel<<<grid, 256, 0, stream>>>(P, in, per_channel, channels, mean_ntt, invstd_ntt, invstd_shoup, out, chunks, per);
    return cudaGetLastError();
}

cudaError_t launch_plain_op(const DeviceParams *P, int n, int K, uint64_t *data, long count, int size,
                               const uint64_t *pl, const uint64_t *pl_sh, int op, cudaStream_t stream) {
    if (count <= 0) return cudaSuccess;
    const long active = (long)(op == 0 ? size : 1) * K * n;
    dim3 grid((unsigned)count, (unsigned)((active / 4 + 255) / 256));
    plain_op_kernel<<<grid, 256, 0, stream>>>(P, data, size, pl, pl_sh, op);
    return cudaGetLastError();
}

#define CRCNN_BEHZ_DISPATCH(KERNEL, GRID, ...)                                                                  \
    do {                                                                                                       \
        if (behz_fold_ok(hp)) {                                                                                \
            if (hp.K == 2 && hp.S == 3) KERNEL<2, 3, true><<<GRID, 128, 0, stream>>>(hp, __VA_ARGS__);          \
            else if (hp.K == 4 && hp.S == 5) KERNEL<4, 5, true><<<GRID, 128, 0, stream>>>(hp, __VA_ARGS__);     \
            else if (hp.K == 8 && hp.S == 9) KERNEL<8, 9, true><<<GRID, 128, 0, stream>>>(hp, __VA_ARGS__);     \
            else KERNEL<0, 0, true><<<GRID, 128, 0, stream>>>(hp, __VA_ARGS__);                                 \
        } else {                                                                                               \
            if (hp.K == 2 && hp.S == 3) KERNEL<2, 3, false><<<GRID, 128, 0, stream>>>(hp, __VA_ARGS__);         \
            else if (hp.K == 4 && hp.S == 5) KERNEL<4, 5, false><<<GRID, 128, 0, stream>>>(hp, __VA_ARGS__);    \
            else if (hp.K == 8 && hp.S == 9) KERNEL<8, 9, false><<<GRID, 128, 0, stream>>>(hp, __VA_ARGS__);    \
            else KERNEL<0, 0, false><<<GRID, 128, 0, stream>>>(hp, __VA_ARGS__);                                \
        }                                                                                                      \
    } while (0)

bool behz_fold_ok(const DeviceParams &hp) {
    static const int env = [] { const char *e = getenv("CRCNN_BEHZ_FOLD"); return e ? atoi(e) : 1; }();
    if (!env) return false;
    for (int i = 0; i < hp.K + hp.S; i++)
        if (!fold128_make(hp.tab[i].mod.q).ok) return false;
    return true;
}

cudaError_t launch_behz_lift(const DeviceParams &P, int n, const uint64_t *in, const uint64_t *in_ntt, long count, uint64_t *ext,
                                cudaStream_t stream, bool ninv_in) {
    if (count <= 0) return cudaSuccess;
    if (!ninv_in && !in_ntt) return cudaErrorInvalidValue;
    DeviceParams scaled;
    if (!ninv_in) {
        scaled = P;
        std::memcpy(scaled.mt_inv_qhat, P.mt_inv_qhat_n, sizeof scaled.mt_inv_qhat);
    }
    const DeviceParams &hp = ninv_in ? P : scaled;
    const unsigned grid = (unsigned)(count * 2 * (n / 128));
    CRCNN_BEHZ_DISPATCH(behz_lift_kernel, grid, in, in_ntt, ext);
    return cudaGetLastError();
}

cudaError_t launch_behz_floor(const DeviceParams &P, int n, const uint64_t *prod, long count, uint64_t *out,
                                 cudaStream_t stream, bool ninv_in) {
    if (count <= 0) return cudaSuccess;
    DeviceParams scaled;
    if (!ninv_in) {
        scaled = P;
        std::memcpy(scaled.fl_c, P.fl_c_n, sizeof scaled.fl_c);
        std::memcpy(scaled.fl_T, P.fl_T_n, sizeof scaled.fl_T);
    }
    const DeviceParams &hp = ninv_in ? P : scaled;
    const unsigned grid = (unsigned)(count * 3 * (n / 128));
    CRCNN_BEHZ_DISPATCH(behz_floor_kernel, grid, prod, out);
    return cudaGetLastError();
}

__global__ void __launch_bounds__(256)
canonicalize_kernel(const DeviceParams *__restrict__ P, uint64_t *__restrict__ data, long words) {
    const long w = (long)blockIdx.x * 256 + threadIdx.x;
    if (w >= words) return;
    const int n = P->n, K = P->K;
    const uint64_t q = P->tab[(w / n) % K].mod.q;
    uint64_t v = data[w];
    v = v >= 2 * q ? v - 2 * q : v;
    data[w] = v >= q ? v - q : v;
}

cudaError_t launch_canonicalize(const DeviceParams *P, uint64_t *data, long words, cudaStream_t stream) {
    if (words <= 0) return cudaSuccess;
    canonicalize_kernel<<<(unsigned)((words + 255) / 256), 256, 0, stream>>>(P, data, words);
    return cudaGetLastError();
}

__global__ void __launch_bounds__(256)
strip_pad_kernel(const uint64_t *__restrict__ src, uint64_t *__restrict__ dst, int n) {
    const long row = blockIdx.x;
    const uint64_t *s = src + row * (n + 1);
    uint64_t *d = dst + row * n;
    for (int i = threadIdx.x; i < n; i += 256) d[i] = __ldg(s + i);
}

cudaError_t launch_strip_pad(const uint64_t *src_padded, uint64_t *dst, long rows, int n, cudaStream_t stream) {
    if (rows <= 0) return cudaSuccess;
    strip_pad_kernel<<<(unsigned)rows, 256, 0, stream>>>(src_padded, dst, n);
    return cudaGetLastError();
}

__global__ void imad_probe_kernel(int iters, uint64_t *sink) {
    uint64_t a = 0x9E3779B97F4A7C15ULL * (threadIdx.x + 1), b = 0xD1B54A32D192ED03ULL + blockIdx.x;
    Acc7 acc[8];
#pragma unroll
    for (int i = 0; i < 8; i++) acc[i] = acc7_from((uint64_t)i);
    for (int it = 0; it < iters; it++) {
#pragma unroll
        for (int i = 0; i < 8; i++) mac7(acc[i], a + i, b);
        a += acc[0].a3;
        b ^= acc[7].a0;
    }
    uint64_t s = 0;
#pragma unroll
    for (int i = 0; i < 8; i++) { U128 v = acc7_value(acc[i]); s += v.lo ^ v.hi; }
    if (s == 0x1234567) sink[0] = s;
}

cudaError_t launch_imad_probe(int blocks, int threads, int iters, uint64_t *sink, cudaStream_t stream) {
    imad_probe_kernel<<<blocks, threads, 0, stream>>>(iters, sink);
    return cudaGetLastError();
}

__global__ void imad_wide_probe_kernel(int iters, uint64_t *sink) {
    uint32_t a = 0x9E3779B9u * (threadIdx.x + 1), b = 0x85EBCA6Bu + blockIdx.x;
    uint64_t acc[16];
#pragma unroll
    for (int i = 0; i < 16; i++) acc[i] = (uint64_t)i * 0x100000001ull;
    for (int it = 0; it < iters; it++) {
#pragma unroll
        for (int i = 0; i < 16; i++)
            asm volatile("mad.wide.u32 %0, %1, %2, %0;" : "+l"(acc[i]) : "r"(a + i), "r"(b));
    }
    uint64_t s = 0;
#pragma unroll
    for (int i = 0; i < 16; i++) s ^= acc[i];
    if (s == 0x1234567) sink[0] = s;
}

cudaError_t launch_imad_wide_probe(int blocks, int threads, int iters, uint64_t *sink, cudaStream_t stream) {
    imad_wide_probe_kernel<<<blocks, threads, 0, stream>>>(iters, sink);
    return cudaGetLastError();
}

}
```

### crcnn_b200/csrc/kernels.cuh

```cuda
#pragma once
#include <cuda_runtime.h>
#include <cstdint>
#include "params.h"

namespace crcnn {

cudaError_t launch_ntt(const DeviceParams *P, int logn, uint64_t *data, long npolys, int slot_base, int slot_count,
                       bool inverse, cudaStream_t stream);

cudaError_t launch_ntt_grouped(const DeviceParams *P, int logn, uint64_t *data, long npolys, int slot_base, int slot_count,
                               bool inverse, int group_polys, int group_off, cudaStream_t stream, const uint64_t *src = nullptr,
                               const uint64_t *addend = nullptr, int add_group = 1, int add_stride = 1, bool ninv = true);

cudaError_t launch_plain_expand(const DeviceParams *P, int logn, int K, const uint32_t *offsets, const uint32_t *idx,
                                const uint64_t *val, long first, long count, int mode, bool to_ntt, uint64_t *out,
                                cudaStream_t stream);

struct MacArgs {
    const uint64_t *x;
    const uint64_t *w;
    const uint64_t *bias;
    const int *in_index;
    uint64_t *out;
    int R, M, Npos, Pimg, Mtotal, m0;
    int K, n;
    int chunk_terms;
};
cudaError_t launch_mac(const DeviceParams *P, const MacArgs &a, cudaStream_t stream);

cudaError_t launch_pool(const DeviceParams *P, int n, int K, const uint64_t *in, const int *in_index, int Nout, int R,
                        const uint64_t *scale_ntt, const uint64_t *scale_shoup, bool sum_fits_64, uint64_t *out,
                        cudaStream_t stream, int per_channel = 1, int channels = 0, const uint64_t *sub = nullptr);
cudaError_t launch_pool_bn_consts(const DeviceParams *P, const uint64_t *S, const uint64_t *V, const uint64_t *M, long words,
                                  uint64_t *C, uint64_t *D, cudaStream_t stream);

cudaError_t launch_bn(const DeviceParams *P, int n, int K, const uint64_t *in, long count, int per_channel, int channels,
                      const uint64_t *mean_ntt, const uint64_t *invstd_ntt, const uint64_t *invstd_shoup, uint64_t *out,
                      cudaStream_t stream);

struct TapMulArgs {
    const uint64_t *in;
    const int *in_index;
    int R;
    const uint64_t *sub;
    const uint32_t *t_off;
    const uint32_t *t_idx;
    const uint64_t *t_val;
    int per_channel, channels;
    uint64_t *out;
    long nout;
};
cudaError_t launch_tapmul(const DeviceParams *P, int n, int K, const TapMulArgs &a, cudaStream_t stream);

cudaError_t launch_fold_affine(const DeviceParams *P, uint64_t *data, long rows, long poly_words, int group, const uint64_t *C,
                               const uint64_t *D, cudaStream_t stream);
cudaError_t launch_fold_fc_input_affine(const DeviceParams *P, uint64_t *W, int out_dim, int in_dim, long poly_words, int per_channel,
                                        const uint64_t *C, const uint64_t *D, uint64_t *Bias, cudaStream_t stream);
cudaError_t launch_scale_small(const DeviceParams *P, uint64_t *data, long words, int times, cudaStream_t stream);
cudaError_t launch_shoup_companion(const DeviceParams *P, const uint64_t *data, long words, uint64_t *out, cudaStream_t stream);

cudaError_t launch_plain_op(const DeviceParams *P, int n, int K, uint64_t *data, long count, int size, const uint64_t *pl, const uint64_t *pl_sh, int op,
                            cudaStream_t stream);

cudaError_t launch_behz_lift(const DeviceParams &hp, int n, const uint64_t *in, const uint64_t *in_ntt, long count, uint64_t *ext,
                             cudaStream_t stream, bool ninv_in = true);
cudaError_t launch_behz_floor(const DeviceParams &hp, int n, const uint64_t *prod, long count, uint64_t *out, cudaStream_t stream,
                              bool ninv_in = true);
bool behz_fold_ok(const DeviceParams &hp);

struct RelinArgs {
    const uint64_t *in3;
    const uint64_t *evk;
    long key_off[MAXK];
    int digits[MAXK];
    int dbc;
    uint64_t *out;
    long count;
    uint64_t *dsc, *dig, *acc;
};
cudaError_t launch_ntt_inv_tensor(const DeviceParams *P, int logn, const uint64_t *ext, const uint64_t *qntt, long count, int KS, uint64_t *prod,
                                  bool fold, bool ninv, cudaStream_t stream);

cudaError_t launch_relin(const DeviceParams *P, int logn, int K, const RelinArgs &a, cudaStream_t stream);
cudaError_t launch_relin_finish(const DeviceParams *P, int n, int K, const RelinArgs &a, cudaStream_t stream);

cudaError_t launch_canonicalize(const DeviceParams *P, uint64_t *data, long words, cudaStream_t stream);

cudaError_t launch_strip_pad(const uint64_t *src_padded, uint64_t *dst, long rows, int n, cudaStream_t stream);

cudaError_t launch_imad_probe(int blocks, int threads, int iters, uint64_t *sink, cudaStream_t stream);
cudaError_t launch_imad_wide_probe(int blocks, int threads, int iters, uint64_t *sink, cudaStream_t stream);

}
```

### crcnn_b200/csrc/params.cpp

```cpp
#include "params.h"
#include <cmath>
#include <stdexcept>

namespace crcnn {

typedef unsigned __int128 u128;

static const uint64_t kAuxPrimes[] = {
    0x1fffffffffb40001ULL, 0x1fffffffff500001ULL, 0x1fffffffff380001ULL, 0x1fffffffff000001ULL,
    0x1ffffffffef00001ULL, 0x1ffffffffee80001ULL, 0x1ffffffffeb40001ULL, 0x1ffffffffe780001ULL,
    0x1ffffffffe600001ULL, 0x1ffffffffe4c0001ULL};
static const uint64_t kMsk = 0x1fffffffffe00001ULL;
static const uint64_t kMtilde = 1ULL << 32;

static int bits_of(uint64_t v) {
    int b = 0;
    for (; v; v >>= 1) b++;
    return b;
}

Mod make_mod(uint64_t q) {
    u128 ones = ~(u128)0;
    u128 quo = ones / q;
    if (ones % q == (u128)(q - 1)) quo++;
// ... 23 lines not shown
    }
    if (r0 != 1) throw std::invalid_argument("inv_mod: operand not invertible");
    if (s0 < 0) s0 += q;
    return (uint64_t)s0;
}

bool minimal_primitive_root(uint64_t degree, const Mod &m, uint64_t &root) {
    if ((m.q - 1) % degree) return false;
    uint64_t cof = (m.q - 1) / degree, start = 0;
    for (uint64_t g = 2; g < 1u << 16 && !start; g++) {
        uint64_t c = pow_mod(g, cof, m);
        if (pow_mod(c, degree / 2, m) == m.q - 1) start = c;
    }
    if (!start) return false;
    uint64_t step = mulmod(start, start, m), cur = start, best = start;
    for (uint64_t i = 0; i < degree / 2; i++) {
        if (cur < best) best = cur;
        cur = mulmod(cur, step, m);
    }
    root = best;
    return true;
}

static uint32_t bit_reverse(uint32_t x, int bits) {
    uint32_t r = 0;
    for (int i = 0; i < bits; i++, x >>= 1) r = (r << 1) | (x & 1);
    return r;
}

static uint64_t product_mod(const uint64_t *v, int count, int skip, const Mod &m) {
    uint64_t r = 1 % m.q;
    for (int i = 0; i < count; i++)
        if (i != skip) r = mulmod(r, v[i] % m.q, m);
    return r;
}

static void build_tables(HostParams &hp, int slot, int logn, const Mod &m) {
    int n = 1 << logn;
    uint64_t psi;
    if (!minimal_primitive_root(2ull * n, m, psi))
        throw std::invalid_argument("modulus " + std::to_string(m.q) + " has no primitive 2n-th root of unity");
    uint64_t psi_inv = inv_mod(psi, m.q);
    auto &w = hp.w[slot], &wp = hp.wp[slot], &iw = hp.iw[slot], &iwp = hp.iwp[slot];
    auto &iwf = hp.iwf[slot], &iwfp = hp.iwfp[slot];
    w.assign(n, 0); wp.assign(n, 0); iw.assign(n, 0); iwp.assign(n, 0); iwf.assign(n, 0); iwfp.assign(n, 0);
    uint64_t pw = 1, ipw = 1;
    for (int i = 0; i < n; i++) {
        uint32_t r = bit_reverse((uint32_t)i, logn);
        w[r] = pw;
        iw[r] = (ipw & 1) ? (uint64_t)(((u128)ipw + m.q) >> 1) : (ipw >> 1);
        iwf[r] = ipw;
        pw = mulmod(pw, psi, m);
        ipw = mulmod(ipw, psi_inv, m);
    }
    for (int i = 0; i < n; i++) {
        wp[i] = (uint64_t)((((u128)w[i]) << 64) / m.q);
        iwp[i] = (uint64_t)((((u128)iw[i]) << 64) / m.q);
        iwfp[i] = (uint64_t)((((u128)iwf[i]) << 64) / m.q);
    }
    hp.d.tab[slot].ninv = inv_mod((uint64_t)n % m.q, m.q);
    hp.d.tab[slot].ninvp = (uint64_t)((((u128)hp.d.tab[slot].ninv) << 64) / m.q);
    hp.roots[slot] = psi;
}

HostParams derive_params(int n, int K, const uint64_t *q, uint64_t t) {
    int logn = 0;
    while ((1 << logn) < n) logn++;
    if (n < 1024 || n > 16384 || (1 << logn) != n) throw std::invalid_argument("n must be a power of two in [1024, 16384]");
    if (K < 1 || K > MAXK) throw std::invalid_argument("coefficient modulus count must be in [1, 8]");
    if (t < 2) throw std::invalid_argument("plain modulus must be at least 2");
    int total_bits = 0;
    for (int i = 0; i < K; i++) {
        if (bits_of(q[i]) > 60 || q[i] < 2) throw std::invalid_argument("coefficient primes must be at most 60 bits");
        if (q[i] <= t) throw std::invalid_argument("plain modulus must be smaller than every coefficient prime (fast plain lift)");
        for (int j = 0; j < i; j++)
            if (q[i] == q[j]) throw std::invalid_argument("coefficient primes must be distinct");
        total_bits += bits_of(q[i]);
    }
    HostParams hp;
    DeviceParams &d = hp.d;
    d.n = n; d.logn = logn; d.K = K; d.t = t; d.half = (t + 1) >> 1;
    d.L = K + ((32 + bits_of(t) + total_bits >= 61 * K + 61) ? 1 : 0);
    d.S = d.L + 1;
    int slots = K + d.S;
    hp.w.resize(slots); hp.wp.resize(slots); hp.iw.resize(slots); hp.iwp.resize(slots); hp.iwf.resize(slots); hp.iwfp.resize(slots); hp.roots.resize(slots);

    std::vector<uint64_t> bsk(d.S);
    for (int i = 0; i < d.L; i++) bsk[i] = kAuxPrimes[i];
    bsk[d.L] = kMsk;
    for (int i = 0; i < K; i++) { d.tab[i].mod = make_mod(q[i]); build_tables(hp, i, logn, d.tab[i].mod); }
    for (int k = 0; k < d.S; k++) { d.tab[K + k].mod = make_mod(bsk[k]); build_tables(hp, K + k, logn, d.tab[K + k].mod); }
    for (int s = 0; s < slots; s++) d.t_mod[s] = t % d.tab[s].mod.q;
    hp.tf.resize(K);
    const int skip = sparse_skip_stages(logn);
    for (int j = 0; j < K; j++) {
        const Mod &m = d.tab[j].mod;
        hp.tf[j].assign((size_t)1 << skip, 0);
        for (int b = 0; b < (1 << skip); b++) {
            uint64_t c = 1;
            for (int s = 0; s < skip; s++) {
                uint64_t w = hp.w[j][((size_t)1 << s) + (b >> (skip - s))];
                if ((b >> (skip - 1 - s)) & 1) w = negmod(w, m.q);
                c = mulmod(c, w, m);
            }
            hp.tf[j][b] = c;
        }
    }

    Mod mt = make_mod(kMtilde), msk = make_mod(kMsk), tm = make_mod(t);
    uint64_t rho = product_mod(q, K, -1, tm);
    for (int j = 0; j < K; j++) {
        const Mod &m = d.tab[j].mod;
        d.rho[j] = rho % m.q;
        d.delta[j] = mulmod(negmod(d.rho[j], m.q), inv_mod(t % m.q, m.q), m);
        d.lift_inc[j] = m.q - t;
        d.inv_qhat[j] = inv_mod(product_mod(q, K, j, m), m.q);
        d.mt_inv_qhat[j] = mulmod(d.inv_qhat[j], kMtilde % m.q, m);
        d.qhat_mod_mt[j] = product_mod(q, K, j, mt);
        d.M_mod_q[j] = product_mod(bsk.data(), d.L, -1, m);
        d.neg_M_mod_q[j] = m.q - d.M_mod_q[j];
        for (int i = 0; i < d.L; i++) d.Mhat_mod_q[j][i] = product_mod(bsk.data(), d.L, i, m);
    }
    d.neg_inv_q_mod_mt = (kMtilde - inv_mod(product_mod(q, K, -1, mt), kMtilde)) % kMtilde;
    for (int k = 0; k < d.S; k++) {
        const Mod &m = d.tab[K + k].mod;
        for (int i = 0; i < K; i++) d.qhat_mod_bsk[k][i] = product_mod(q, K, i, m);
        d.q_mod_bsk[k] = product_mod(q, K, -1, m);
        d.inv_q_mod_bsk[k] = inv_mod(d.q_mod_bsk[k], m.q);
        d.inv_mt_mod_bsk[k] = inv_mod(kMtilde % m.q, m.q);
    }
    for (int i = 0; i < d.L; i++) {
        const Mod &m = d.tab[K + i].mod;
        d.inv_Mhat[i] = inv_mod(product_mod(bsk.data(), d.L, i, m), m.q);
        d.Mhat_mod_msk[i] = product_mod(bsk.data(), d.L, i, msk);
    }
    d.inv_M_mod_msk = inv_mod(product_mod(bsk.data(), d.L, -1, msk), kMsk);
    for (int j = 0; j < K; j++) d.fl_c[j] = mulmod(t % d.tab[j].mod.q, d.inv_qhat[j], d.tab[j].mod);
    for (int k = 0; k < d.S; k++) {
        const Mod &m = d.tab[K + k].mod;
        const uint64_t fold = k < d.L ? mulmod(d.inv_q_mod_bsk[k], d.inv_Mhat[k], m) : d.inv_q_mod_bsk[k];
        d.lift_b[k] = mulmod(d.q_mod_bsk[k], d.inv_mt_mod_bsk[k], m);
        d.fl_T[k] = mulmod(t % m.q, fold, m);
        for (int i = 0; i < K; i++) {
            d.lift_a[k][i] = mulmod(d.qhat_mod_bsk[k][i], d.inv_mt_mod_bsk[k], m);
            d.fl_N[k][i] = negmod(mulmod(d.qhat_mod_bsk[k][i], fold, m), m.q);
        }
    }
    for (int i = 0; i < d.L; i++) d.fl_P[i] = mulmod(d.Mhat_mod_msk[i], d.inv_M_mod_msk, msk);
    for (int j = 0; j < K; j++) {
        d.mt_inv_qhat_n[j] = mulmod(d.mt_inv_qhat[j], d.tab[j].ninv, d.tab[j].mod);
        d.fl_c_n[j] = mulmod(d.fl_c[j], d.tab[j].ninv, d.tab[j].mod);
    }
    for (int k = 0; k < d.S; k++) d.fl_T_n[k] = mulmod(d.fl_T[k], d.tab[K + k].ninv, d.tab[K + k].mod);
    return hp;
}

static void encode_integer_b3(int64_t v, uint64_t t, std::vector<uint32_t> &idx, std::vector<uint64_t> &val) {
    bool neg = v < 0;
    uint64_t mag = neg ? (uint64_t)(-v) : (uint64_t)v;
    for (uint32_t pos = 0; mag; pos++) {
        uint64_t rem = mag % 3;
        int digit = rem == 0 ? 0 : (rem == 1 ? 1 : -1);
        mag = (mag + 1) / 3;
        if (neg) digit = -digit;
        if (digit) { idx.push_back(pos); val.push_back(digit > 0 ? 1 : t - 1); }
    }
}

void encode_fractional_sparse(double value, int n, uint64_t t, std::vector<uint32_t> &idx,
                              std::vector<uint64_t> &val) {
    int64_t ip = (int64_t)std::round(value);
    encode_integer_b3(ip, t, idx, val);
    double frac = value - (double)ip;
    if (frac == 0) return;
    for (int i = 0; i < 32; i++) {
        frac *= 3.0;
        int sign = frac >= 0 ? 1 : -1;
        int64_t digit = (int64_t)(sign * std::ceil(std::fabs(frac) - 0.5));
        frac -= (double)digit;
        if (digit) { idx.push_back((uint32_t)(n - 1 - i)); val.push_back(digit > 0 ? t - (uint64_t)digit : (uint64_t)(-digit)); }
    }
}

}
```

### crcnn_b200/csrc/params.h

```cpp
#pragma once
#include <cstdint>
#include <string>
#include <vector>
#include "modarith.cuh"

namespace crcnn {

constexpr int MAXK = 8;
constexpr int MAXS = 10;
constexpr int MAXDIG = 4;

struct NttTable {
    Mod mod;
    const uint64_t *w;
    const uint64_t *iw;
    uint64_t ninv, ninvp;
    const uint64_t *tf;
    const uint64_t *wl;
    const uint64_t *iwl;
};

#if defined(__CUDACC__)
__host__ __device__
#endif
constexpr int sparse_skip_stages(int logn) { return logn == 13 ? 6 : logn == 12 ? 4 : logn == 14 ? 6 : 3; }

struct DeviceParams {
    int n, logn, K, L, S;
    uint64_t t, half;
    NttTable tab[MAXK + MAXS];
    uint64_t delta[MAXK];
    uint64_t rho[MAXK];
    uint64_t lift_inc[MAXK];
    uint64_t inv_qhat[MAXK];
    uint64_t mt_inv_qhat[MAXK];
    uint64_t qhat_mod_bsk[MAXS][MAXK];
    uint64_t qhat_mod_mt[MAXK];
    uint64_t neg_inv_q_mod_mt;
    uint64_t q_mod_bsk[MAXS];
    uint64_t inv_mt_mod_bsk[MAXS];
    uint64_t inv_q_mod_bsk[MAXS];
    uint64_t inv_Mhat[MAXS];
    uint64_t Mhat_mod_q[MAXK][MAXS];
    uint64_t Mhat_mod_msk[MAXS];
    uint64_t inv_M_mod_msk;
    uint64_t M_mod_q[MAXK];
    uint64_t neg_M_mod_q[MAXK];
    uint64_t t_mod[MAXK + MAXS];
    uint64_t lift_a[MAXS][MAXK];
    uint64_t lift_b[MAXS];
    uint64_t fl_c[MAXK];
    uint64_t fl_T[MAXS];
    uint64_t fl_N[MAXS][MAXK];
    uint64_t fl_P[MAXS];
    uint64_t mt_inv_qhat_n[MAXK];
    uint64_t fl_c_n[MAXK];
    uint64_t fl_T_n[MAXS];
};

struct HostParams {
    DeviceParams d{};
    std::vector<std::vector<uint64_t>> w, wp, iw, iwp;
    std::vector<std::vector<uint64_t>> iwf, iwfp;
    std::vector<uint64_t> roots;
    std::vector<std::vector<uint64_t>> tf;
};

HostParams derive_params(int n, int K, const uint64_t *q, uint64_t t);

Mod make_mod(uint64_t q);
uint64_t inv_mod(uint64_t a, uint64_t q);
uint64_t pow_mod(uint64_t a, uint64_t e, const Mod &m);
bool minimal_primitive_root(uint64_t degree, const Mod &m, uint64_t &root);

void encode_fractional_sparse(double value, int n, uint64_t t, std::vector<uint32_t> &idx,
                              std::vector<uint64_t> &val);

}
```

### crcnn_b200/csrc/relin32.cu

```cuda
#include "relin32.cuh"
#include "kernels.cuh"
#include "devcfg.cuh"
#include "modarith.cuh"
#include <cmath>
#include <cstdlib>
#include <vector>

namespace crcnn {
namespace {

const uint32_t kAuxPrimes[R32_MAXP] = {1073643521u, 1073479681u, 1073184769u, 1073053697u};

uint32_t mulm(uint32_t a, uint32_t b, uint32_t p) { return (uint32_t)((uint64_t)a * b % p); }
uint32_t powm(uint32_t a, uint64_t e, uint32_t p) {
    uint32_t r = 1;
    for (; e; e >>= 1, a = mulm(a, a, p))
        if (e & 1) r = mulm(r, a, p);
    return r;
}
uint32_t invm(uint32_t a, uint32_t p) { return powm(a % p, p - 2, p); }
uint32_t shoup_companion(uint32_t w, uint32_t p) { return (uint32_t)(((uint64_t)w << 32) / p); }
uint32_t bitrev32(uint32_t v, int bits) {
    uint32_t r = 0;
    for (int i = 0; i < bits; i++) r |= ((v >> i) & 1u) << (bits - 1 - i);
// ... 351 lines not shown
            if (d0 + 16 < D) {
#pragma unroll
                for (int t = 0; t < T; t++)
#pragma unroll
                    for (int o = 0; o < OC; o++) a[t][o] = red64_32(a[t][o], mu, p);
            }
        }
#pragma unroll
        for (int t = 0; t < T; t++)
            if (c0 + t < cte) {
                uint32_t *ap = acc + (((c0 + t) * OC) * S3 + s) * n + e;
#pragma unroll
                for (int o = 0; o < OC; o++) ap[(long)o * S3 * n] = red64_32(a[t][o], mu, p);
            }
    }
}

__device__ __forceinline__ void cp_async16(void *smem_dst, const void *gsrc) {
    asm volatile("cp.async.cg.shared.global [%0], [%1], 16;" ::"r"((uint32_t)__cvta_generic_to_shared(smem_dst)), "l"(gsrc));
}
__device__ __forceinline__ void cp_async_commit() { asm volatile("cp.async.commit_group;"); }
template <int N>
__device__ __forceinline__ void cp_async_wait() { asm volatile("cp.async.wait_group %0;" ::"n"(N)); }

template <int D, int OC>
__global__ void __launch_bounds__(32 * OC)
r32_mac_reg_kernel(const uint32_t *__restrict__ dig, const uint32_t *__restrict__ keys, const Relin32Consts *__restrict__ cp, int n,
                   long count, int cpb, uint32_t *__restrict__ acc) {
    constexpr int EW = 64, CPS = 2, NS = 6, SW = CPS * D * EW;
    extern __shared__ uint4 sm32v[];
    uint32_t *sm = reinterpret_cast<uint32_t *>(sm32v);
    const int el = threadIdx.x % EW, og = threadIdx.x / EW;
    const int e0 = blockIdx.x * EW;
    const int s = blockIdx.y, S3 = cp->S3;
    const long ctb = (long)blockIdx.z * cpb;
    const long cte = min(ctb + cpb, count);
    const int nst = (int)((cte - ctb + CPS - 1) / CPS);
    const uint32_t p = cp->p[s];
    const uint64_t mu = cp->mu[s];
    uint32_t k0[D], k1[D];
    {
        const uint32_t *kg = keys + ((long)s * D * OC + og * 2) * n + e0 + el;
#pragma unroll
        for (int d = 0; d < D; d++) {
            k0[d] = __ldg(kg + (long)d * OC * n);
            k1[d] = __ldg(kg + (long)d * OC * n + n);
        }
    }
    const int cd = threadIdx.x / 16, cpart = threadIdx.x % 16;
    auto issue = [&](int st) {
        if (st < nst) {
            uint32_t *dst = sm + (st % NS) * SW + cd * EW + cpart * 4;
#pragma unroll
            for (int u = 0; u < CPS; u++) {
                const long ct = min(ctb + (long)st * CPS + u, count - 1);
                cp_async16(dst + u * D * EW, dig + ((ct * D + cd) * S3 + s) * n + e0 + cpart * 4);
            }
        }
        cp_async_commit();
    };
#pragma unroll
    for (int st = 0; st < NS - 1; st++) issue(st);
    for (int st = 0; st < nst; st++) {
        cp_async_wait<NS - 2>();
        __syncthreads();
        issue(st + NS - 1);
        const uint32_t *tile = sm + (st % NS) * SW + el;
        uint64_t a[CPS][2];
#pragma unroll
        for (int u = 0; u < CPS; u++) {
            a[u][0] = 0;
            a[u][1] = 0;
        }
#pragma unroll
        for (int d = 0; d < D; d++) {
#pragma unroll
            for (int u = 0; u < CPS; u++) {
                const uint32_t x = tile[(u * D + d) * EW];
                madwide(a[u][0], x, k0[d]);
                madwide(a[u][1], x, k1[d]);
            }
            if (D > 16 && d == 15) {
#pragma unroll
                for (int u = 0; u < CPS; u++) {
                    a[u][0] = red64_32(a[u][0], mu, p);
                    a[u][1] = red64_32(a[u][1], mu, p);
                }
            }
        }
#pragma unroll
        for (int u = 0; u < CPS; u++) {
            const long ct = ctb + (long)st * CPS + u;
            if (ct < cte) {
                uint32_t *ap = acc + ((ct * OC + og * 2) * S3 + s) * n + e0 + el;
                ap[0] = red64_32(a[u][0], mu, p);
                ap[(long)S3 * n] = red64_32(a[u][1], mu, p);
            }
        }
    }
}

template <int LOGN>
__global__ void __launch_bounds__(Plan32<LOGN>::THREADS, Plan32<LOGN>::MIN_CTAS)
r32_intt_kernel(const Relin32Consts *__restrict__ cp, uint32_t *__restrict__ acc) {
    extern __shared__ uint4 sm32v[];
    uint32_t *sm32 = reinterpret_cast<uint32_t *>(sm32v);
    constexpr int N = 1 << LOGN;
    const long b = blockIdx.x;
    const int s = (int)(b % cp->S3);
    const uint32_t p = cp->p[s];
    const uint2 *iw = cp->iw[s];
    uint32_t *poly = acc + b * N;
    for (int i = threadIdx.x * 4; i < N; i += Plan32<LOGN>::THREADS * 4)
        *reinterpret_cast<uint4 *>(sm32 + pad32(i)) = *reinterpret_cast<const uint4 *>(poly + i);
    __syncthreads();
    ntt32_inverse<LOGN>(sm32, iw, cp->iwl[s], p);
    store32_canonical<LOGN, 2>(sm32, poly, p);
}

struct CrtConsts {
    uint32_t p[R32_MAXP], half[R32_MAXP], ginv[R32_MAXP][R32_MAXP], ginvp[R32_MAXP][R32_MAXP];
    uint64_t c[R32_MAXP], csh[R32_MAXP], Pmodq, q;
};
template <int S3>
__device__ __forceinline__ uint64_t crt_one(const uint32_t (&r)[R32_MAXP], const CrtConsts &k) {
    uint32_t a[S3];
#pragma unroll
    for (int s = 0; s < S3; s++) {
        uint32_t t = r[s];
#pragma unroll
        for (int i = 0; i < s; i++) {
            const uint32_t ai = csub(a[i], k.p[s]);
            t = csub(shoup32(t + k.p[s] - ai, k.ginv[s][i], k.ginvp[s][i], k.p[s]), k.p[s]);
        }
        a[s] = t;
    }
    uint64_t v = a[0];
    bool neg = false, decided = false;
#pragma unroll
    for (int s = S3 - 1; s >= 0; s--) {
        if (s > 0) v += mulshoup_lazy((uint64_t)a[s], k.c[s], k.csh[s], k.q);
        if (!decided && a[s] != k.half[s]) { neg = a[s] > k.half[s]; decided = true; }
    }
    v = v >= 4 * k.q ? v - 4 * k.q : v;
    v = v >= 2 * k.q ? v - 2 * k.q : v;
    v = v >= k.q ? v - k.q : v;
    if (neg) v = submod(v, k.Pmodq, k.q);
    return v;
}

template <int S3>
__global__ void __launch_bounds__(256)
r32_crt_kernel(const DeviceParams *__restrict__ P, const Relin32Consts *__restrict__ cp, const uint32_t *__restrict__ acc,
               const uint64_t *__restrict__ in3, uint64_t *__restrict__ out) {
    const int n = P->n, K = P->K;
    const int e = (blockIdx.y * 256 + threadIdx.x) * 2;
    const int o = (int)(blockIdx.x % (unsigned)(2 * K));
    const long ct = blockIdx.x / (unsigned)(2 * K);
    const int pi = o / K, j = o % K;
    CrtConsts k;
#pragma unroll
    for (int s = 0; s < S3; s++) {
        k.p[s] = cp->p[s];
        k.half[s] = cp->half[s];
        k.c[s] = cp->cmodq[j][s];
        k.csh[s] = cp->cmodq_sh[j][s];
#pragma unroll
        for (int i = 0; i < s; i++) {
            k.ginv[s][i] = cp->ginv[s][i];
            k.ginvp[s][i] = cp->ginvp[s][i];
        }
    }
    k.Pmodq = cp->Pmodq[j];
    k.q = P->tab[j].mod.q;
    const uint32_t *r = acc + ((ct * 2 * K + o) * S3) * n + e;
    uint32_t r0[R32_MAXP], r1[R32_MAXP];
#pragma unroll
    for (int s = 0; s < S3; s++) {
        const uint2 v = __ldg(reinterpret_cast<const uint2 *>(r + (long)s * n));
        r0[s] = v.x;
        r1[s] = v.y;
    }
    const long w = (long)j * n + e;
    const ulonglong2 c = __ldg(reinterpret_cast<const ulonglong2 *>(in3 + (ct * 3 + pi) * (long)K * n + w));
    ulonglong2 res;
    res.x = addmod(c.x, crt_one<S3>(r0, k), k.q);
    res.y = addmod(c.y, crt_one<S3>(r1, k), k.q);
    *reinterpret_cast<ulonglong2 *>(out + (ct * 2 + pi) * (long)K * n + w) = res;
}

template <int LOGN, int S3>
__global__ void __launch_bounds__(Plan32<LOGN>::THREADS, 2)
r32_intt_crt_kernel(const DeviceParams *__restrict__ P, const Relin32Consts *__restrict__ cp, const uint32_t *__restrict__ acc,
                    const uint64_t *__restrict__ in3, uint64_t *__restrict__ out) {
    extern __shared__ uint4 sm32v[];
    uint32_t *sm32 = reinterpret_cast<uint32_t *>(sm32v);
    constexpr int N = 1 << LOGN, SW = Plan32<LOGN>::SMEM_WORDS;
    const int K = P->K;
    const long b = blockIdx.x;
    const int o = (int)(b % (2 * K));
    const long ct = b / (2 * K);
    const int pi = o / K, j = o % K;
#pragma unroll
    for (int s = 0; s < S3; s++) {
        const uint32_t *poly = acc + (b * S3 + s) * N;
        for (int i = threadIdx.x * 4; i < N; i += Plan32<LOGN>::THREADS * 4)
            *reinterpret_cast<uint4 *>(sm32 + s * SW + pad32(i)) = __ldg(reinterpret_cast<const uint4 *>(poly + i));
    }
    __syncthreads();
#pragma unroll
    for (int s = 0; s < S3; s++) ntt32_inverse<LOGN>(sm32 + s * SW, cp->iw[s], cp->iwl[s], cp->p[s]);
    CrtConsts k;
#pragma unroll
    for (int s = 0; s < S3; s++) {
        k.p[s] = cp->p[s];
        k.half[s] = cp->half[s];
        k.c[s] = cp->cmodq[j][s];
        k.csh[s] = cp->cmodq_sh[j][s];
#pragma unroll
        for (int i = 0; i < s; i++) {
            k.ginv[s][i] = cp->ginv[s][i];
            k.ginvp[s][i] = cp->ginvp[s][i];
        }
    }
    k.Pmodq = cp->Pmodq[j];
    k.q = P->tab[j].mod.q;
    const uint64_t *cin = in3 + (ct * 3 + pi) * (long)K * N + (long)j * N;
    uint64_t *dst = out + (ct * 2 + pi) * (long)K * N + (long)j * N;
    for (int e = threadIdx.x * 2; e < N; e += Plan32<LOGN>::THREADS * 2) {
        uint32_t r0[R32_MAXP], r1[R32_MAXP];
#pragma unroll
        for (int s = 0; s < S3; s++) {
            const uint2 v = *reinterpret_cast<const uint2 *>(sm32 + s * SW + pad32(e));
            r0[s] = csub(v.x, k.p[s]);
            r1[s] = csub(v.y, k.p[s]);
        }
        const ulonglong2 c = __ldg(reinterpret_cast<const ulonglong2 *>(cin + e));
        ulonglong2 res;
        res.x = addmod(c.x, crt_one<S3>(r0, k), k.q);
        res.y = addmod(c.y, crt_one<S3>(r1, k), k.q);
        *reinterpret_cast<ulonglong2 *>(dst + e) = res;
    }
}

template <int LOGN>
void configure32() {
    static DeviceOnce once;
    if (!once.first()) return;
    const int smem = Plan32<LOGN>::SMEM_WORDS * 4;
    cudaFuncSetAttribute(r32_digits_kernel<LOGN>, cudaFuncAttributeMaxDynamicSharedMemorySize, smem);
    cudaFuncSetAttribute(r32_key_kernel<LOGN>, cudaFuncAttributeMaxDynamicSharedMemorySize, smem);
    cudaFuncSetAttribute(r32_intt_kernel<LOGN>, cudaFuncAttributeMaxDynamicSharedMemorySize, smem);
    cudaFuncSetAttribute(r32_digits_kernel<LOGN>, cudaFuncAttributePreferredSharedMemoryCarveout, cudaSharedmemCarveoutMaxShared);
    cudaFuncSetAttribute(r32_intt_kernel<LOGN>, cudaFuncAttributePreferredSharedMemoryCarveout, cudaSharedmemCarveoutMaxShared);
}

template <int T, int OC, int EW>
cudaError_t launch_mac(const uint32_t *dig, const Relin32 &r, int n, long count, int cpb, unsigned gz, size_t bytes_per_coeff, uint32_t *acc,
                       cudaStream_t stream) {
    const size_t smem = bytes_per_coeff * EW;
    cudaError_t e = cudaFuncSetAttribute(r32_mac_kernel<T, OC, EW>, cudaFuncAttributeMaxDynamicSharedMemorySize, (int)smem);
    if (e != cudaSuccess) return e;
    r32_mac_kernel<T, OC, EW><<<dim3((unsigned)(n / EW), (unsigned)r.c.S3, gz), 256, smem, stream>>>(dig, r.keys, r.dc, n, count, cpb, acc);
    return cudaGetLastError();
}

template <int D, int OC>
cudaError_t launch_mac_reg(const uint32_t *dig, const Relin32 &r, int n, long count, int cpb, unsigned gz, uint32_t *acc, cudaStream_t stream) {
    constexpr size_t smem = (size_t)6 * 2 * D * 64 * 4;
    static DeviceOnce once;
    if (once.first()) {
        cudaError_t e = cudaFuncSetAttribute(r32_mac_reg_kernel<D, OC>, cudaFuncAttributeMaxDynamicSharedMemorySize, (int)smem);
        if (e != cudaSuccess) return e;
        cudaFuncSetAttribute(r32_mac_reg_kernel<D, OC>, cudaFuncAttributePreferredSharedMemoryCarveout, cudaSharedmemCarveoutMaxShared);
    }
    r32_mac_reg_kernel<D, OC><<<dim3((unsigned)(n / 64), (unsigned)r.c.S3, gz), 32 * OC, smem, stream>>>(dig, r.keys, r.dc, n, count, cpb, acc);
    return cudaGetLastError();
}

template <int LOGN>
cudaError_t run_t(const DeviceParams *dP, int K, const Relin32 &r, const uint64_t *in3, uint64_t *out, long count, void *scratch,
                  cudaStream_t stream) {
    using Pl = Plan32<LOGN>;
    constexpr int N = 1 << LOGN;
    configure32<LOGN>();
    const Relin32Consts &c = r.c;
    const size_t smem = Pl::SMEM_WORDS * 4;
    uint32_t *dig = (uint32_t *)scratch;
    uint32_t *acc = dig + (size_t)count * c.D * c.S3 * N;
    uint16_t *planes = (uint16_t *)(acc + (size_t)count * 2 * K * c.S3 * N);
    r32_scale_kernel<<<dim3((unsigned)count, (unsigned)((long)K * N / 512)), 256, 0, stream>>>(dP, r.dc, in3, planes);
    r32_digits_kernel<LOGN><<<(unsigned)(count * c.D * c.S3), Pl::THREADS, smem, stream>>>(planes, r.dc, dig);
    {
        const int cpb = 128;
        const unsigned gz = (unsigned)((count + cpb - 1) / cpb);
        const size_t ksmem = (size_t)c.D * 2 * K * 4;
        cudaError_t e = cudaSuccess;
        const bool generic = std::getenv("CRCNN_R32_GENERIC_MAC") != nullptr;
        if (!generic && c.D == 4 * K && K == 1) e = launch_mac_reg<4, 2>(dig, r, N, count, cpb, gz, acc, stream);
        else if (!generic && c.D == 4 * K && K == 2) e = launch_mac_reg<8, 4>(dig, r, N, count, cpb, gz, acc, stream);
        else if (!generic && c.D == 4 * K && K == 4) e = launch_mac_reg<16, 8>(dig, r, N, count, cpb, gz, acc, stream);
        else if (!generic && c.D == 4 * K && K == 8) e = launch_mac_reg<32, 16>(dig, r, N, count, cpb, gz, acc, stream);
        else
        switch (2 * K) {
            case 2: e = launch_mac<4, 2, 64>(dig, r, N, count, cpb, gz, ksmem, acc, stream); break;
            case 4: e = launch_mac<4, 4, 64>(dig, r, N, count, cpb, gz, ksmem, acc, stream); break;
            case 8: e = launch_mac<4, 8, 64>(dig, r, N, count, cpb, gz, ksmem, acc, stream); break;
            case 16: e = launch_mac<2, 16, 32>(dig, r, N, count, cpb, gz, ksmem, acc, stream); break;
            default: e = cudaErrorInvalidValue;
        }
        if (e != cudaSuccess) return e;
    }
    if constexpr (LOGN <= 13) {
        static const bool fused = !(std::getenv("CRCNN_R32_FUSED") && std::atoi(std::getenv("CRCNN_R32_FUSED")) == 0);
        if (fused && c.S3 == 3) {
            static DeviceOnce once3;
            const int smem3 = 3 * Pl::SMEM_WORDS * 4;
            if (once3.first()) {
                cudaFuncSetAttribute(r32_intt_crt_kernel<LOGN, 3>, cudaFuncAttributeMaxDynamicSharedMemorySize, smem3);
                cudaFuncSetAttribute(r32_intt_crt_kernel<LOGN, 3>, cudaFuncAttributePreferredSharedMemoryCarveout, cudaSharedmemCarveoutMaxShared);
            }
            r32_intt_crt_kernel<LOGN, 3><<<(unsigned)(count * 2 * K), Pl::THREADS, smem3, stream>>>(dP, r.dc, acc, in3, out);
            return cudaGetLastError();
        }
    }
    r32_intt_kernel<LOGN><<<(unsigned)(count * 2 * K * c.S3), Pl::THREADS, smem, stream>>>(r.dc, acc);
    const dim3 gc((unsigned)(count * 2 * K), (unsigned)(N / 512));
    if (c.S3 == 2) r32_crt_kernel<2><<<gc, 256, 0, stream>>>(dP, r.dc, acc, in3, out);
    else if (c.S3 == 3) r32_crt_kernel<3><<<gc, 256, 0, stream>>>(dP, r.dc, acc, in3, out);
    else r32_crt_kernel<4><<<gc, 256, 0, stream>>>(dP, r.dc, acc, in3, out);
    return cudaGetLastError();
}

template <int LOGN>
cudaError_t build_keys_t(const uint64_t *coef, const KeyMap &km, const Relin32 &r, int K, cudaStream_t stream) {
    configure32<LOGN>();
    r32_key_kernel<LOGN><<<(unsigned)((long)r.c.D * 2 * K * r.c.S3), Plan32<LOGN>::THREADS, Plan32<LOGN>::SMEM_WORDS * 4, stream>>>(
        coef, km, r.dc, K, r.keys);
    return cudaGetLastError();
}

}

bool relin32_applicable(int n, int K, const uint64_t *q, const int *digits, int dbc, Relin32Consts &c) {
    if (n < 1024 || n > 16384 || (n & (n - 1))) return false;
    if (dbc < 1 || dbc > 16) return false;
    if (K != 1 && K != 2 && K != 4 && K != 8) return false;
    c = Relin32Consts{};
    c.dbc = dbc;
    uint64_t qmax = 0;
    for (int i = 0; i < K; i++) {
        if (q[i] > qmax) qmax = q[i];
        c.dfirst[i] = c.D;
        for (int k = 0; k < digits[i]; k++) {
            if (c.D >= 32) return false;
            c.dprime[c.D] = (unsigned char)i;
            c.dshift[c.D] = (unsigned char)(k * dbc);
            c.D++;
        }
    }
    if (c.D == 0) return false;
    const double need = 1.0 + std::log2((double)c.D) + std::log2((double)n) + (double)dbc + std::log2((double)qmax);
    double have = 0;
    for (int s = 0; s < R32_MAXP; s++) {
        have += std::log2((double)kAuxPrimes[s]);
        if (have > need + 1e-3 && s + 1 >= 2) { c.S3 = s + 1; break; }
    }
    if (c.S3 == 0) return false;
    for (int s = 0; s < c.S3; s++) {
        c.p[s] = kAuxPrimes[s];
        c.mu[s] = (uint64_t)((((unsigned __int128)1) << 64) / kAuxPrimes[s]);
        c.half[s] = (kAuxPrimes[s] - 1) / 2;
        for (int k = 0; k < s; k++) {
            c.ginv[s][k] = invm(kAuxPrimes[k] % kAuxPrimes[s], kAuxPrimes[s]);
            c.ginvp[s][k] = shoup_companion(c.ginv[s][k], kAuxPrimes[s]);
        }
    }
    for (int j = 0; j < K; j++) {
        unsigned __int128 prod = 1;
        for (int s = 0; s < c.S3; s++) {
            c.cmodq[j][s] = (uint64_t)prod;
            c.cmodq_sh[j][s] = (uint64_t)((prod << 64) / q[j]);
            prod = prod * kAuxPrimes[s] % q[j];
        }
        c.Pmodq[j] = (uint64_t)prod;
    }
    return true;
}

cudaError_t relin32_build(const DeviceParams *dP, int logn, int K, const uint64_t *q, const uint64_t *evk_dev, const long *key_off,
                          long total_polys, Relin32 &r, cudaStream_t stream) {
    (void)q;
    const int n = 1 << logn;
    Relin32Consts &c = r.c;
    std::vector<uint2> host((size_t)4 * c.S3 * n);
    const int NG = n >> 5;
    KeyMap km{};
    for (int s = 0; s < c.S3; s++) {
        const uint32_t p = c.p[s];
        uint32_t psi = 0;
        for (uint32_t z = 2; z < 1000 && !psi; z++) {
            const uint32_t cand = powm(z, (p - 1) / (2u * n), p);
            if (powm(cand, n, p) == p - 1) psi = cand;
        }
        if (!psi) return cudaErrorInvalidValue;
        const uint32_t psi_inv = invm(psi, p);
        uint32_t pw = 1, ipw = 1;
        uint2 *w = host.data() + (size_t)(4 * s) * n, *iw = w + n, *wl = iw + n, *iwl = wl + n;
        for (int i = 0; i < n; i++) {
            const uint32_t rv = bitrev32((uint32_t)i, logn);
            w[rv] = make_uint2(pw, shoup_companion(pw, p));
            iw[rv] = make_uint2(ipw, shoup_companion(ipw, p));
            pw = mulm(pw, psi, p);
            ipw = mulm(ipw, psi_inv, p);
        }
        km.ninv[s] = invm((uint32_t)n, p);
        for (int G = 0; G < NG; G++) {
            wl[30 * NG + G] = w[NG + G];
            iwl[30 * NG + G] = iw[(n >> 5) + G];
            for (int st = 1; st < 5; st++)
                for (int l2 = 0; l2 < (1 << (st - 1)); l2++) {
                    const size_t at = 2 * ((size_t)((1 << (st - 1)) - 1 + l2) * NG + G);
                    wl[at] = w[((NG + G) << st) + 2 * l2];
                    wl[at + 1] = w[((NG + G) << st) + 2 * l2 + 1];
                }
            for (int st = 0; st < 4; st++)
                for (int l2 = 0; l2 < (1 << (3 - st)); l2++) {
                    const size_t at = 2 * ((size_t)(16 - (16 >> st) + l2) * NG + G);
                    const int idx = ((n >> 1) >> st) + (G << (4 - st)) + 2 * l2;
                    iwl[at] = iw[idx];
                    iwl[at + 1] = iw[idx + 1];
                }
        }
    }
    cudaError_t e = cudaMalloc((void **)&r.tables, host.size() * sizeof(uint2));
    if (e != cudaSuccess) return e;
    e = cudaMemcpyAsync(r.tables, host.data(), host.size() * sizeof(uint2), cudaMemcpyHostToDevice, stream);
    if (e != cudaSuccess) return e;
    e = cudaStreamSynchronize(stream);
    if (e != cudaSuccess) return e;
    for (int s = 0; s < c.S3; s++) {
        c.w[s] = r.tables + (size_t)(4 * s) * n;
        c.iw[s] = r.tables + (size_t)(4 * s + 1) * n;
        c.wl[s] = r.tables + (size_t)(4 * s + 2) * n;
        c.iwl[s] = r.tables + (size_t)(4 * s + 3) * n;
    }
    for (int i = 0; i < MAXK; i++) km.key_off[i] = key_off[i];
    e = cudaMalloc((void **)&r.dc, sizeof(Relin32Consts));
    if (e != cudaSuccess) return e;
    e = cudaMemcpyAsync(r.dc, &c, sizeof(Relin32Consts), cudaMemcpyHostToDevice, stream);
    if (e != cudaSuccess) return e;
    const size_t words = (size_t)total_polys * K * n;
    uint64_t *coef = nullptr;
    e = cudaMalloc((void **)&coef, words * 8);
    if (e != cudaSuccess) return e;
    e = cudaMalloc((void **)&r.keys, (size_t)c.S3 * c.D * 2 * K * n * 4);
    if (e != cudaSuccess) { cudaFree(coef); return e; }
    e = cudaMemcpyAsync(coef, evk_dev, words * 8, cudaMemcpyDeviceToDevice, stream);
    if (e == cudaSuccess) e = launch_ntt(dP, logn, coef, total_polys * K, 0, K, true, stream);
    if (e == cudaSuccess) {
        switch (logn) {
            case 10: e = build_keys_t<10>(coef, km, r, K, stream); break;
            case 11: e = build_keys_t<11>(coef, km, r, K, stream); break;
            case 12: e = build_keys_t<12>(coef, km, r, K, stream); break;
            case 13: e = build_keys_t<13>(coef, km, r, K, stream); break;
            case 14: e = build_keys_t<14>(coef, km, r, K, stream); break;
            default: e = cudaErrorInvalidValue;
        }
    }
    if (e == cudaSuccess) e = cudaStreamSynchronize(stream);
    cudaFree(coef);
    return e;
}

void relin32_free(Relin32 &r) {
    if (r.keys) cudaFree(r.keys);
    if (r.tables) cudaFree(r.tables);
    if (r.dc) cudaFree(r.dc);
    r.dc = nullptr;
    r.keys = nullptr;
    r.tables = nullptr;
}

size_t relin32_scratch_bytes(int n, int K, const Relin32Consts &c) {
    return (size_t)c.D * c.S3 * n * 4 + (size_t)2 * K * c.S3 * n * 4 + (size_t)c.D * n * 2;
}

cudaError_t relin32_run(const DeviceParams *dP, int logn, int K, const Relin32 &r, const uint64_t *in3, uint64_t *out, long count,
                        void *scratch, cudaStream_t stream) {
    if (count <= 0) return cudaSuccess;
    switch (logn) {
        case 10: return run_t<10>(dP, K, r, in3, out, count, scratch, stream);
        case 11: return run_t<11>(dP, K, r, in3, out, count, scratch, stream);
        case 12: return run_t<12>(dP, K, r, in3, out, count, scratch, stream);
        case 13: return run_t<13>(dP, K, r, in3, out, count, scratch, stream);
        case 14: return run_t<14>(dP, K, r, in3, out, count, scratch, stream);
        default: return cudaErrorInvalidValue;
    }
}

}
```

### crcnn_b200/csrc/relin32.cuh

```cuda
#pragma once
#include <cuda_runtime.h>
#include <cstdint>
#include "params.h"

namespace crcnn {

constexpr int R32_MAXP = 4;

struct Relin32Consts {
    int S3;
    int D;
    int dbc;
    uint32_t p[R32_MAXP];
    uint64_t mu[R32_MAXP];
    const uint2 *w[R32_MAXP];
    const uint2 *iw[R32_MAXP];
    const uint2 *wl[R32_MAXP], *iwl[R32_MAXP];
    uint32_t ginv[R32_MAXP][R32_MAXP];
    uint32_t ginvp[R32_MAXP][R32_MAXP];
    uint32_t half[R32_MAXP];
    uint64_t cmodq[MAXK][R32_MAXP];
    uint64_t cmodq_sh[MAXK][R32_MAXP];
    uint64_t Pmodq[MAXK];
    unsigned char dprime[32], dshift[32];
    int dfirst[MAXK];
};

struct Relin32 {
    Relin32Consts c;
    uint32_t *keys = nullptr;
    uint2 *tables = nullptr;
    Relin32Consts *dc = nullptr;
};

bool relin32_applicable(int n, int K, const uint64_t *q, const int *digits, int dbc, Relin32Consts &c);

cudaError_t relin32_build(const DeviceParams *dP, int logn, int K, const uint64_t *q, const uint64_t *evk_dev, const long *key_off,
                          long total_polys, Relin32 &r, cudaStream_t stream);
void relin32_free(Relin32 &r);

size_t relin32_scratch_bytes(int n, int K, const Relin32Consts &c);

cudaError_t relin32_run(const DeviceParams *dP, int logn, int K, const Relin32 &r, const uint64_t *in3, uint64_t *out, long count,
                        void *scratch, cudaStream_t stream);

}
```

Baseline: 40.97.

## Fuse BEHZ floor with relinearization digit decomposition in square_forward

Adds a fused square+relinearize path. The BEHZ floor kernel writes the c0/c1 components straight into the size-2 output and, for the c2 component, multiplies by inv_qhat through precomputed constants and emits the 16-bit digit planes that relin32 consumes. This removes the intermediate size-3 tensor, the separate scale kernel pass and its global memory round trip. The relin CRT kernels now accumulate in place on the output. The cost is extra precomputed parameters and a more complex floor kernel, guarded by an env flag.

```diff
diff --git a/crcnn_b200/csrc/engine.cu b/crcnn_b200/csrc/engine.cu
--- a/crcnn_b200/csrc/engine.cu
+++ b/crcnn_b200/csrc/engine.cu
@@ -102,6 +102,7 @@
     int relin_mode = 1;
     int tcn_mode = 1;
     int sq_lean = 1;
+    int sq_fuse = 1;
     int tcn_preshift = 1;
     int tcn_fold = 1;
     size_t tc_scratch_bytes = 12ull << 30;
@@ -603,6 +604,7 @@
     if (const char *e = getenv("CRCNN_TCN_FOLD")) c->tcn_fold = atoi(e);
     if (const char *e = getenv("CRCNN_TCN2_PRESHIFT")) c->tcn_preshift = atoi(e);
     if (const char *e = getenv("CRCNN_SQ_LEAN")) c->sq_lean = atoi(e);
+    if (const char *e = getenv("CRCNN_SQ_FUSE")) c->sq_fuse = atoi(e);
     cudaMemPool_t pool;
     if (cudaDeviceGetDefaultMemPool(&pool, device) == cudaSuccess) {
         uint64_t thr = UINT64_MAX;
@@ -1503,62 +1505,86 @@
     return CRCNN_OK;
 }
 
+struct SquareScratch {
+    bool have_ntt, lean, fold, copy_ninv;
+    uint64_t *ext = nullptr, *prod = nullptr, *coef = nullptr;
+};
+
+static size_t square_bytes_per_ct(const crcnn_ctx *ctx) { return (size_t)5 * (ctx->K + ctx->S) * ctx->n * 8; }
+
+static int square_scratch_alloc(crcnn_ctx *ctx, const crcnn_tensor *in, long step, SquareScratch &sq) {
+    sq.have_ntt = in->ntt != 0;
+    sq.lean = ctx->sq_lean != 0;
+    sq.fold = sq.lean && behz_fold_ok(ctx->hp.d);
+    sq.copy_ninv = !(sq.lean && sq.have_ntt);
+    const size_t KS = ctx->K + ctx->S, n = ctx->n, pw = poly_words(ctx);
+    int rc = dev_alloc(ctx, (size_t)step * 2 * KS * n * 8, (void **)&sq.ext);
+    if (!rc) rc = dev_alloc(ctx, (size_t)step * 3 * KS * n * 8, (void **)&sq.prod);
+    if (!rc && sq.have_ntt) rc = dev_alloc(ctx, (size_t)step * 2 * pw * 8, (void **)&sq.coef);
+    return rc;
+}
+
+static void square_scratch_free(crcnn_ctx *ctx, SquareScratch &sq) {
+    dev_free(ctx, sq.coef);
+    dev_free(ctx, sq.ext); dev_free(ctx, sq.prod);
+}
+
+static cudaError_t square_products(crcnn_ctx *ctx, const SquareScratch &sq, const uint64_t *src, long cur) {
+    const int KS = ctx->K + ctx->S;
+    const size_t n = ctx->n;
+    const bool have_ntt = sq.have_ntt;
+    uint64_t *ext = sq.ext, *coef = sq.coef;
+    cudaError_t e = cudaSuccess;
+    if (have_ntt) {
+        ProfScope ps(ctx, KC_NTT_INV, 2 * lp_bytes(ctx, (double)cur * 2 * ctx->K), lp_bfly(ctx, (double)cur * 2 * ctx->K));
+        e = launch_ntt_grouped(ctx->dP, ctx->logn, coef, cur * 2 * ctx->K, 0, ctx->K, true, ctx->K, 0, ctx->stream, src,
+                               nullptr, 1, 1, sq.copy_ninv);
+    }
+    if (e == cudaSuccess) { ProfScope ps(ctx, KC_BEHZ_LIFT, lp_bytes(ctx, (double)cur * 2 * (ctx->K + (have_ntt ? ctx->S : KS))), (double)cur * 2 * n * ctx->S * (ctx->K + 1)); e = launch_behz_lift(ctx->hp.d, ctx->n, have_ntt ? coef : src, have_ntt ? src : nullptr, cur, ext, ctx->stream, sq.copy_ninv); }
+    if (e == cudaSuccess) {
+        if (have_ntt) {
+            ProfScope ps(ctx, KC_NTT_FWD, 2 * lp_bytes(ctx, (double)cur * 2 * ctx->S), lp_bfly(ctx, (double)cur * 2 * ctx->S));
+            e = launch_ntt_grouped(ctx->dP, ctx->logn, ext, cur * 2 * ctx->S, ctx->K, ctx->S, false, KS, ctx->K, ctx->stream);
+        } else {
+            ProfScope ps(ctx, KC_NTT_FWD, 2 * lp_bytes(ctx, (double)cur * 2 * KS), lp_bfly(ctx, (double)cur * 2 * KS));
+            e = launch_ntt(ctx->dP, ctx->logn, ext, cur * 2 * KS, 0, KS, false, ctx->stream);
+        }
+    }
+    if (e == cudaSuccess) {
+        ProfScope ps(ctx, KC_SQ_TENSOR, lp_bytes(ctx, (double)cur * 5 * KS), lp_bfly(ctx, (double)cur * 3 * KS));
+        e = launch_ntt_inv_tensor(ctx->dP, ctx->logn, ext, have_ntt ? src : nullptr, cur, KS, sq.prod, sq.fold, !sq.lean, ctx->stream);
+    }
+    return e;
+}
+
 int crcnn_square(crcnn_ctx *ctx, crcnn_tensor *in, crcnn_tensor **out3) {
     if (!ctx) return CRCNN_ERR_INVALID_ARGUMENT;
     REQUIRE(in && out3, "null argument");
     REQUIRE(in->size == 2, "square expects size-2 ciphertexts");
     CU(cudaSetDevice(ctx->device));
-    const bool have_ntt = in->ntt != 0;
-    const bool lean = ctx->sq_lean != 0, fold = lean && behz_fold_ok(ctx->hp.d), copy_ninv = !(lean && have_ntt);
     crcnn_tensor *o = nullptr;
     int rc = new_tensor(ctx, in->count, 3, 0, &o);
     if (rc) return rc;
     const int KS = ctx->K + ctx->S;
-    const size_t n = ctx->n, pw = poly_words(ctx);
-    const long step = std::max<long>(1, std::min<long>(in->count, (long)((2ull << 30) / (5 * (size_t)KS * n * 8))));
-    uint64_t *ext = nullptr, *prod = nullptr, *coef = nullptr;
-    rc = dev_alloc(ctx, (size_t)step * 2 * KS * n * 8, (void **)&ext);
-    if (!rc) rc = dev_alloc(ctx, (size_t)step * 3 * KS * n * 8, (void **)&prod);
-    if (!rc && have_ntt) rc = dev_alloc(ctx, (size_t)step * 2 * pw * 8, (void **)&coef);
-    if (rc) { crcnn_tensor_free(ctx, o); return rc; }
+    const size_t pw = poly_words(ctx);
+    const long step = std::max<long>(1, std::min<long>(in->count, (long)((2ull << 30) / square_bytes_per_ct(ctx))));
+    SquareScratch sq;
+    rc = square_scratch_alloc(ctx, in, step, sq);
+    if (rc) { square_scratch_free(ctx, sq); crcnn_tensor_free(ctx, o); return rc; }
     for (long c0 = 0; c0 < in->count && !rc; c0 += step) {
         const long cur = std::min<long>(step, in->count - c0);
-        const uint64_t *src = in->d + c0 * 2 * pw;
-        cudaError_t e = cudaSuccess;
-        if (have_ntt) {
-            ProfScope ps(ctx, KC_NTT_INV, 2 * lp_bytes(ctx, (double)cur * 2 * ctx->K), lp_bfly(ctx, (double)cur * 2 * ctx->K));
-            e = launch_ntt_grouped(ctx->dP, ctx->logn, coef, cur * 2 * ctx->K, 0, ctx->K, true, ctx->K, 0, ctx->stream, src,
-                                   nullptr, 1, 1, copy_ninv);
-        }
-        if (e == cudaSuccess) { ProfScope ps(ctx, KC_BEHZ_LIFT, lp_bytes(ctx, (double)cur * 2 * (ctx->K + (have_ntt ? ctx->S : KS))), (double)cur * 2 * n * ctx->S * (ctx->K + 1)); e = launch_behz_lift(ctx->hp.d, ctx->n, have_ntt ? coef : src, have_ntt ? src : nullptr, cur, ext, ctx->stream, copy_ninv); }
-        if (e == cudaSuccess) {
-            if (have_ntt) {
-                ProfScope ps(ctx, KC_NTT_FWD, 2 * lp_bytes(ctx, (double)cur * 2 * ctx->S), lp_bfly(ctx, (double)cur * 2 * ctx->S));
-                e = launch_ntt_grouped(ctx->dP, ctx->logn, ext, cur * 2 * ctx->S, ctx->K, ctx->S, false, KS, ctx->K, ctx->stream);
-            } else {
-                ProfScope ps(ctx, KC_NTT_FWD, 2 * lp_bytes(ctx, (double)cur * 2 * KS), lp_bfly(ctx, (double)cur * 2 * KS));
-                e = launch_ntt(ctx->dP, ctx->logn, ext, cur * 2 * KS, 0, KS, false, ctx->stream);
-            }
-        }
-        if (e == cudaSuccess) {
-            ProfScope ps(ctx, KC_SQ_TENSOR, lp_bytes(ctx, (double)cur * 5 * KS), lp_bfly(ctx, (double)cur * 3 * KS));
-            e = launch_ntt_inv_tensor(ctx->dP, ctx->logn, ext, have_ntt ? src : nullptr, cur, KS, prod, fold, !lean, ctx->stream);
-        }
+        cudaError_t e = square_products(ctx, sq, in->d + c0 * 2 * pw, cur);
         if (e == cudaSuccess) { ProfScope ps(ctx, KC_BEHZ_FLOOR, lp_bytes(ctx, (double)cur * 3 * (KS + ctx->K)),
-                                                     (double)cur * 3 * n * (ctx->S * (ctx->K + 1) + ctx->S + ctx->K * ctx->S)); e = launch_behz_floor(ctx->hp.d, ctx->n, prod, cur, o->d + c0 * 3 * pw, ctx->stream, !lean); }
+                                                     (double)cur * 3 * ctx->n * (ctx->S * (ctx->K + 1) + ctx->S + ctx->K * ctx->S)); e = launch_behz_floor(ctx->hp.d, ctx->n, sq.prod, cur, o->d + c0 * 3 * pw, ctx->stream, !sq.lean); }
         if (e != cudaSuccess) rc = fail(ctx, CRCNN_ERR_CUDA, cudaGetErrorString(e));
     }
-    dev_free(ctx, coef);
-    dev_free(ctx, ext); dev_free(ctx, prod);
+    square_scratch_free(ctx, sq);
     if (rc) { crcnn_tensor_free(ctx, o); return rc; }
     *out3 = o;
     return CRCNN_OK;
 }
 
-int crcnn_relinearize(crcnn_ctx *ctx, crcnn_tensor *in3, crcnn_evk *evk, crcnn_tensor **out2) {
-    if (!ctx) return CRCNN_ERR_INVALID_ARGUMENT;
-    REQUIRE(in3 && evk && out2, "null argument");
-    REQUIRE(in3->size == 3, "relinearize expects size-3 ciphertexts");
+static int relin_check_keys(crcnn_ctx *ctx, const crcnn_evk *evk, int *total) {
     int total_digits = 0;
     for (int i = 0; i < ctx->K; i++) {
         int bits = 0; for (uint64_t v = ctx->hp.d.tab[i].mod.q; v; v >>= 1) bits++;
@@ -1566,8 +1592,19 @@
         total_digits += evk->digits[i];
     }
     REQUIRE(total_digits <= 63, "too many key digits for 128-bit lazy accumulation");
-    CU(cudaSetDevice(ctx->device));
-    int rc = ensure_domain(ctx, in3, 0);
+    *total = total_digits;
+    return CRCNN_OK;
+}
+
+int crcnn_relinearize(crcnn_ctx *ctx, crcnn_tensor *in3, crcnn_evk *evk, crcnn_tensor **out2) {
+    if (!ctx) return CRCNN_ERR_INVALID_ARGUMENT;
+    REQUIRE(in3 && evk && out2, "null argument");
+    REQUIRE(in3->size == 3, "relinearize expects size-3 ciphertexts");
+    int total_digits = 0;
+    int rc = relin_check_keys(ctx, evk, &total_digits);
+    if (rc) return rc;
+    CU(cudaSetDevice(ctx->device));
+    rc = ensure_domain(ctx, in3, 0);
     if (rc) return rc;
     crcnn_tensor *o = nullptr;
     rc = new_tensor(ctx, in3->count, 2, 0, &o);
@@ -1624,12 +1661,57 @@
 
 int crcnn_square_forward(crcnn_ctx *ctx, crcnn_tensor *in, crcnn_evk *evk, crcnn_tensor **out) {
     if (!ctx) return CRCNN_ERR_INVALID_ARGUMENT;
-    crcnn_tensor *t3 = nullptr;
-    int rc = crcnn_square(ctx, in, &t3);
-    if (rc) return rc;
-    rc = crcnn_relinearize(ctx, t3, evk, out);
-    crcnn_tensor_free(ctx, t3);
-    return rc;
+    if (!(ctx->sq_fuse && in && evk && out && in->size == 2 && evk->has_r32 && ctx->relin_mode == 1)) {
+        crcnn_tensor *t3 = nullptr;
+        int rc = crcnn_square(ctx, in, &t3);
+        if (rc) return rc;
+        rc = crcnn_relinearize(ctx, t3, evk, out);
+        crcnn_tensor_free(ctx, t3);
+        return rc;
+    }
+    int total_digits = 0;
+    int rc = relin_check_keys(ctx, evk, &total_digits);
+    if (rc) return rc;
+    CU(cudaSetDevice(ctx->device));
+    const Relin32Consts &c = evk->r32.c;
+    crcnn_tensor *o = nullptr;
+    rc = new_tensor(ctx, in->count, 2, 0, &o);
+    if (rc) return rc;
+    const int K = ctx->K, KS = K + ctx->S;
+    const size_t n = ctx->n, pw = poly_words(ctx);
+    const size_t relin_per_ct = relin32_scratch_bytes(ctx->n, K, c);
+    const long step = std::max<long>(1, std::min<long>({in->count, (long)((2ull << 30) / square_bytes_per_ct(ctx)),
+                                                        (long)((2ull << 30) / relin_per_ct)}));
+    SquareScratch sq;
+    void *rscratch = nullptr;
+    rc = square_scratch_alloc(ctx, in, step, sq);
+    if (!rc) rc = dev_alloc(ctx, (size_t)step * relin_per_ct, &rscratch);
+    if (rc) { dev_free(ctx, rscratch); square_scratch_free(ctx, sq); crcnn_tensor_free(ctx, o); return rc; }
+    FloorDigits fd{};
+    fd.D = c.D; fd.dbc = c.dbc;
+    for (int i = 0; i < K; i++) { fd.dfirst[i] = c.dfirst[i]; fd.ndig[i] = evk->digits[i]; }
+    for (long c0 = 0; c0 < in->count && !rc; c0 += step) {
+        const long cur = std::min<long>(step, in->count - c0);
+        uint64_t *dst = o->d + c0 * 2 * pw;
+        cudaError_t e = square_products(ctx, sq, in->d + c0 * 2 * pw, cur);
+        if (e == cudaSuccess) {
+            ProfScope ps(ctx, KC_BEHZ_FLOOR, lp_bytes(ctx, (double)cur * (3 * KS + 2 * K)) + (double)cur * c.D * n * 2,
+                         (double)cur * 3 * n * (ctx->S * (K + 1) + ctx->S + K * ctx->S));
+            fd.planes = relin32_planes(rscratch, ctx->n, K, c, cur);
+            e = launch_behz_floor_digits(ctx->hp.d, ctx->n, sq.prod, cur, dst, fd, ctx->stream, !sq.lean);
+        }
+        if (e == cudaSuccess) {
+            ProfScope ps(ctx, KC_RELIN32, lp_bytes(ctx, (double)cur * 4 * K) + (double)cur * c.D * n * 2,
+                         lp_bfly(ctx, (double)cur * (c.D + 2 * K) * c.S3));
+            e = relin32_run(ctx->dP, ctx->logn, K, evk->r32, nullptr, dst, cur, rscratch, ctx->stream);
+        }
+        if (e != cudaSuccess) rc = fail(ctx, CRCNN_ERR_CUDA, cudaGetErrorString(e));
+    }
+    dev_free(ctx, rscratch);
+    square_scratch_free(ctx, sq);
+    if (rc) { crcnn_tensor_free(ctx, o); return rc; }
+    *out = o;
+    return CRCNN_OK;
 }
 
 int crcnn_transform_to_ntt(crcnn_ctx *ctx, crcnn_tensor *t) {
diff --git a/crcnn_b200/csrc/host_selftest.cpp b/crcnn_b200/csrc/host_selftest.cpp
--- a/crcnn_b200/csrc/host_selftest.cpp
+++ b/crcnn_b200/csrc/host_selftest.cpp
@@ -135,6 +135,31 @@
             printf("ninv %d ok %d\n", s, ok ? 1 : 0);
             if (!ok) { printf("NINV CONSTANT MISMATCH\n"); return 1; }
         }
+        for (int j = 0; j < d.K; j++) {
+            const uint64_t q = d.tab[j].mod.q, iq = d.inv_qhat[j];
+            auto times_iq = [&](uint64_t c) { return (uint64_t)((u128)c * iq % q); };
+            bool ok = d.M_mod_q_iq[j] < q && d.M_mod_q_iq[j] == times_iq(d.M_mod_q[j]);
+            ok = ok && d.neg_M_mod_q_iq[j] < q && d.neg_M_mod_q_iq[j] == times_iq(d.neg_M_mod_q[j]);
+            for (int i = 0; i < d.L; i++) ok = ok && d.Mhat_mod_q_iq[j][i] < q && d.Mhat_mod_q_iq[j][i] == times_iq(d.Mhat_mod_q[j][i]);
+            const uint64_t msk = d.tab[d.K + d.L].mod.q;
+            for (int it = 0; it < 20000 && ok; it++) {
+                u128 e = 0, e_iq = 0;
+                for (int i = 0; i < d.L; i++) {
+                    x = x * 6364136223846793005ULL + 1442695040888963407ULL;
+                    const uint64_t m = d.tab[d.K + i].mod.q, g = it < 2 ? m - 1 : x % m;
+                    e += (u128)g * d.Mhat_mod_q[j][i] % q;
+                    e_iq += (u128)g * d.Mhat_mod_q_iq[j][i] % q;
+                }
+                y = y * 2862933555777941757ULL + 3037000493ULL;
+                const bool neg = it & 1;
+                const uint64_t alpha = it < 2 ? msk >> 1 : y % (msk >> 1);
+                e += (u128)alpha * (neg ? d.M_mod_q[j] : d.neg_M_mod_q[j]) % q;
+                e_iq += (u128)alpha * (neg ? d.M_mod_q_iq[j] : d.neg_M_mod_q_iq[j]) % q;
+                ok = (uint64_t)(e_iq % q) == times_iq((uint64_t)(e % q));
+            }
+            printf("iqhat %d ok %d\n", j, ok ? 1 : 0);
+            if (!ok) { printf("IQHAT CONSTANT MISMATCH\n"); return 1; }
+        }
         for (int s = 0; s < d.K + d.S; s++) {
             const uint64_t q = d.tab[s].mod.q, nq = 0 - q;
             const uint64_t ws[] = {0, 1, q - 1, q / 2, 0x5555555555555555ULL % q, 0};
diff --git a/crcnn_b200/csrc/kernels.cu b/crcnn_b200/csrc/kernels.cu
--- a/crcnn_b200/csrc/kernels.cu
+++ b/crcnn_b200/csrc/kernels.cu
@@ -762,16 +762,16 @@
     }
 }
 
-template <int KT, int ST, bool FOLD>
-__global__ void __launch_bounds__(128)
-behz_floor_kernel(const __grid_constant__ DeviceParams P, const uint64_t *__restrict__ prod, uint64_t *__restrict__ out) {
+template <int KT, int ST, bool FOLD, bool DIG>
+__device__ __forceinline__ void behz_floor_body(const DeviceParams &P, const uint64_t *__restrict__ prod, uint64_t *__restrict__ out,
+                                                const FloorDigits *fd) {
     const int n = P.n, K = KT ? KT : P.K, S = KT ? ST : P.S, L = S - 1;
     constexpr int KB = KT ? KT : MAXK, SB = KT ? ST : MAXS;
     const int per = n / 128;
     const long poly = blockIdx.x / per;
     const int c = (blockIdx.x % per) * 128 + threadIdx.x;
     const uint64_t *src = prod + poly * (K + S) * n + c;
-    uint64_t *dst = out + poly * K * n + c;
+    uint64_t *dst = out + (DIG ? (poly / 3) * 2 + poly % 3 : poly) * K * n + c;
     uint64_t u[KB], g[SB];
 #pragma unroll
     for (int i = 0; i < KB; i++)
@@ -797,6 +797,23 @@
     const uint64_t alpha = behz_reduce<FOLD>(acc7_value(acc), msk);
     const bool centered_neg = alpha > (msk.q >> 1);
     const uint64_t alpha_mag = centered_neg ? msk.q - alpha : alpha;
+    if (DIG && poly % 3 == 2) {
+        uint16_t *pl = fd->planes + (poly / 3) * fd->D * n + c;
+        const uint32_t mask = (1u << fd->dbc) - 1;
+#pragma unroll
+        for (int j = 0; j < KB; j++)
+            if (j < K) {
+                Acc7 e = acc7_zero();
+#pragma unroll
+                for (int i = 0; i < SB; i++)
+                    if (i < L) mac7(e, g[i], P.Mhat_mod_q_iq[j][i]);
+                mac7(e, alpha_mag, centered_neg ? P.M_mod_q_iq[j] : P.neg_M_mod_q_iq[j]);
+                const uint64_t d = behz_reduce<FOLD>(acc7_value(e), P.tab[j].mod);
+                for (int k = 0; k < fd->ndig[j]; k++)
+                    pl[(long)(fd->dfirst[j] + k) * n] = (uint16_t)((uint32_t)(d >> (k * fd->dbc)) & mask);
+            }
+        return;
+    }
 #pragma unroll
     for (int j = 0; j < KB; j++)
         if (j < K) {
@@ -807,6 +824,19 @@
             mac7(e, alpha_mag, centered_neg ? P.M_mod_q[j] : P.neg_M_mod_q[j]);
             dst[(long)j * n] = behz_reduce<FOLD>(acc7_value(e), P.tab[j].mod);
         }
+}
+
+template <int KT, int ST, bool FOLD>
+__global__ void __launch_bounds__(128)
+behz_floor_kernel(const __grid_constant__ DeviceParams P, const uint64_t *__restrict__ prod, uint64_t *__restrict__ out) {
+    behz_floor_body<KT, ST, FOLD, false>(P, prod, out, nullptr);
+}
+
+template <int KT, int ST, bool FOLD>
+__global__ void __launch_bounds__(128)
+behz_floor_digits_kernel(const __grid_constant__ DeviceParams P, const uint64_t *__restrict__ prod, uint64_t *__restrict__ out2,
+                         const __grid_constant__ FloorDigits fd) {
+    behz_floor_body<KT, ST, FOLD, true>(P, prod, out2, &fd);
 }
 
 __global__ void __launch_bounds__(256)
@@ -1017,18 +1047,32 @@
     return cudaGetLastError();
 }
 
+static const DeviceParams &floor_params(const DeviceParams &P, bool ninv_in, DeviceParams &scaled) {
+    if (ninv_in) return P;
+    scaled = P;
+    std::memcpy(scaled.fl_c, P.fl_c_n, sizeof scaled.fl_c);
+    std::memcpy(scaled.fl_T, P.fl_T_n, sizeof scaled.fl_T);
+    return scaled;
+}
+
 cudaError_t launch_behz_floor(const DeviceParams &P, int n, const uint64_t *prod, long count, uint64_t *out,
                                  cudaStream_t stream, bool ninv_in) {
     if (count <= 0) return cudaSuccess;
     DeviceParams scaled;
-    if (!ninv_in) {
-        scaled = P;
-        std::memcpy(scaled.fl_c, P.fl_c_n, sizeof scaled.fl_c);
-        std::memcpy(scaled.fl_T, P.fl_T_n, sizeof scaled.fl_T);
-    }
-    const DeviceParams &hp = ninv_in ? P : scaled;
+    const DeviceParams &hp = floor_params(P, ninv_in, scaled);
     const unsigned grid = (unsigned)(count * 3 * (n / 128));
     CRCNN_BEHZ_DISPATCH(behz_floor_kernel, grid, prod, out);
+    return cudaGetLastError();
+}
+
+cudaError_t launch_behz_floor_digits(const DeviceParams &P, int n, const uint64_t *prod, long count, uint64_t *out2, const FloorDigits &fd,
+                                     cudaStream_t stream, bool ninv_in) {
+    if (count <= 0) return cudaSuccess;
+    if (fd.dbc < 1 || fd.dbc > 16) return cudaErrorInvalidValue;
+    DeviceParams scaled;
+    const DeviceParams &hp = floor_params(P, ninv_in, scaled);
+    const unsigned grid = (unsigned)(count * 3 * (n / 128));
+    CRCNN_BEHZ_DISPATCH(behz_floor_digits_kernel, grid, prod, out2, fd);
     return cudaGetLastError();
 }
 
diff --git a/crcnn_b200/csrc/kernels.cuh b/crcnn_b200/csrc/kernels.cuh
--- a/crcnn_b200/csrc/kernels.cuh
+++ b/crcnn_b200/csrc/kernels.cuh
@@ -66,6 +66,13 @@
                              cudaStream_t stream, bool ninv_in = true);
 cudaError_t launch_behz_floor(const DeviceParams &hp, int n, const uint64_t *prod, long count, uint64_t *out, cudaStream_t stream,
                               bool ninv_in = true);
+struct FloorDigits {
+    uint16_t *planes;
+    int D, dbc;
+    int dfirst[MAXK], ndig[MAXK];
+};
+cudaError_t launch_behz_floor_digits(const DeviceParams &hp, int n, const uint64_t *prod, long count, uint64_t *out2, const FloorDigits &fd,
+                                     cudaStream_t stream, bool ninv_in = true);
 bool behz_fold_ok(const DeviceParams &hp);
 
 struct RelinArgs {
diff --git a/crcnn_b200/csrc/params.cpp b/crcnn_b200/csrc/params.cpp
--- a/crcnn_b200/csrc/params.cpp
+++ b/crcnn_b200/csrc/params.cpp
@@ -199,6 +199,12 @@
         d.fl_c_n[j] = mulmod(d.fl_c[j], d.tab[j].ninv, d.tab[j].mod);
     }
     for (int k = 0; k < d.S; k++) d.fl_T_n[k] = mulmod(d.fl_T[k], d.tab[K + k].ninv, d.tab[K + k].mod);
+    for (int j = 0; j < K; j++) {
+        const Mod &m = d.tab[j].mod;
+        for (int i = 0; i < d.L; i++) d.Mhat_mod_q_iq[j][i] = mulmod(d.Mhat_mod_q[j][i], d.inv_qhat[j], m);
+        d.M_mod_q_iq[j] = mulmod(d.M_mod_q[j], d.inv_qhat[j], m);
+        d.neg_M_mod_q_iq[j] = mulmod(d.neg_M_mod_q[j], d.inv_qhat[j], m);
+    }
     return hp;
 }
 
diff --git a/crcnn_b200/csrc/params.h b/crcnn_b200/csrc/params.h
--- a/crcnn_b200/csrc/params.h
+++ b/crcnn_b200/csrc/params.h
@@ -56,6 +56,9 @@
     uint64_t mt_inv_qhat_n[MAXK];
     uint64_t fl_c_n[MAXK];
     uint64_t fl_T_n[MAXS];
+    uint64_t Mhat_mod_q_iq[MAXK][MAXS];
+    uint64_t M_mod_q_iq[MAXK];
+    uint64_t neg_M_mod_q_iq[MAXK];
 };
 
 struct HostParams {
diff --git a/crcnn_b200/csrc/relin32.cu b/crcnn_b200/csrc/relin32.cu
--- a/crcnn_b200/csrc/relin32.cu
+++ b/crcnn_b200/csrc/relin32.cu
@@ -527,7 +527,7 @@
 template <int S3>
 __global__ void __launch_bounds__(256)
 r32_crt_kernel(const DeviceParams *__restrict__ P, const Relin32Consts *__restrict__ cp, const uint32_t *__restrict__ acc,
-               const uint64_t *__restrict__ in3, uint64_t *__restrict__ out) {
+               const uint64_t *cin, int csize, uint64_t *out) {
     const int n = P->n, K = P->K;
     const int e = (blockIdx.y * 256 + threadIdx.x) * 2;
     const int o = (int)(blockIdx.x % (unsigned)(2 * K));
@@ -557,7 +557,7 @@
         r1[s] = v.y;
     }
     const long w = (long)j * n + e;
-    const ulonglong2 c = __ldg(reinterpret_cast<const ulonglong2 *>(in3 + (ct * 3 + pi) * (long)K * n + w));
+    const ulonglong2 c = *reinterpret_cast<const ulonglong2 *>(cin + (ct * csize + pi) * (long)K * n + w);
     ulonglong2 res;
     res.x = addmod(c.x, crt_one<S3>(r0, k), k.q);
     res.y = addmod(c.y, crt_one<S3>(r1, k), k.q);
@@ -567,7 +567,7 @@
 template <int LOGN, int S3>
 __global__ void __launch_bounds__(Plan32<LOGN>::THREADS, 2)
 r32_intt_crt_kernel(const DeviceParams *__restrict__ P, const Relin32Consts *__restrict__ cp, const uint32_t *__restrict__ acc,
-                    const uint64_t *__restrict__ in3, uint64_t *__restrict__ out) {
+                    const uint64_t *cin, int csize, uint64_t *out) {
     extern __shared__ uint4 sm32v[];
     uint32_t *sm32 = reinterpret_cast<uint32_t *>(sm32v);
     constexpr int N = 1 << LOGN, SW = Plan32<LOGN>::SMEM_WORDS;
@@ -600,7 +600,7 @@
     }
     k.Pmodq = cp->Pmodq[j];
     k.q = P->tab[j].mod.q;
-    const uint64_t *cin = in3 + (ct * 3 + pi) * (long)K * N + (long)j * N;
+    const uint64_t *cp_in = cin + (ct * csize + pi) * (long)K * N + (long)j * N;
     uint64_t *dst = out + (ct * 2 + pi) * (long)K * N + (long)j * N;
     for (int e = threadIdx.x * 2; e < N; e += Plan32<LOGN>::THREADS * 2) {
         uint32_t r0[R32_MAXP], r1[R32_MAXP];
@@ -610,7 +610,7 @@
             r0[s] = csub(v.x, k.p[s]);
             r1[s] = csub(v.y, k.p[s]);
         }
-        const ulonglong2 c = __ldg(reinterpret_cast<const ulonglong2 *>(cin + e));
+        const ulonglong2 c = *reinterpret_cast<const ulonglong2 *>(cp_in + e);
         ulonglong2 res;
         res.x = addmod(c.x, crt_one<S3>(r0, k), k.q);
         res.y = addmod(c.y, crt_one<S3>(r1, k), k.q);
@@ -663,8 +663,10 @@
     const size_t smem = Pl::SMEM_WORDS * 4;
     uint32_t *dig = (uint32_t *)scratch;
     uint32_t *acc = dig + (size_t)count * c.D * c.S3 * N;
-    uint16_t *planes = (uint16_t *)(acc + (size_t)count * 2 * K * c.S3 * N);
-    r32_scale_kernel<<<dim3((unsigned)count, (unsigned)((long)K * N / 512)), 256, 0, stream>>>(dP, r.dc, in3, planes);
+    uint16_t *planes = relin32_planes(scratch, N, K, c, count);
+    const uint64_t *cin = in3 ? in3 : out;
+    const int csize = in3 ? 3 : 2;
+    if (in3) r32_scale_kernel<<<dim3((unsigned)count, (unsigned)((long)K * N / 512)), 256, 0, stream>>>(dP, r.dc, in3, planes);
     r32_digits_kernel<LOGN><<<(unsigned)(count * c.D * c.S3), Pl::THREADS, smem, stream>>>(planes, r.dc, dig);
     {
         const int cpb = 128;
@@ -695,15 +697,15 @@
                 cudaFuncSetAttribute(r32_intt_crt_kernel<LOGN, 3>, cudaFuncAttributeMaxDynamicSharedMemorySize, smem3);
                 cudaFuncSetAttribute(r32_intt_crt_kernel<LOGN, 3>, cudaFuncAttributePreferredSharedMemoryCarveout, cudaSharedmemCarveoutMaxShared);
             }
-            r32_intt_crt_kernel<LOGN, 3><<<(unsigned)(count * 2 * K), Pl::THREADS, smem3, stream>>>(dP, r.dc, acc, in3, out);
+            r32_intt_crt_kernel<LOGN, 3><<<(unsigned)(count * 2 * K), Pl::THREADS, smem3, stream>>>(dP, r.dc, acc, cin, csize, out);
             return cudaGetLastError();
         }
     }
     r32_intt_kernel<LOGN><<<(unsigned)(count * 2 * K * c.S3), Pl::THREADS, smem, stream>>>(r.dc, acc);
     const dim3 gc((unsigned)(count * 2 * K), (unsigned)(N / 512));
-    if (c.S3 == 2) r32_crt_kernel<2><<<gc, 256, 0, stream>>>(dP, r.dc, acc, in3, out);
-    else if (c.S3 == 3) r32_crt_kernel<3><<<gc, 256, 0, stream>>>(dP, r.dc, acc, in3, out);
-    else r32_crt_kernel<4><<<gc, 256, 0, stream>>>(dP, r.dc, acc, in3, out);
+    if (c.S3 == 2) r32_crt_kernel<2><<<gc, 256, 0, stream>>>(dP, r.dc, acc, cin, csize, out);
+    else if (c.S3 == 3) r32_crt_kernel<3><<<gc, 256, 0, stream>>>(dP, r.dc, acc, cin, csize, out);
+    else r32_crt_kernel<4><<<gc, 256, 0, stream>>>(dP, r.dc, acc, cin, csize, out);
     return cudaGetLastError();
 }
 
@@ -861,6 +863,10 @@
     return (size_t)c.D * c.S3 * n * 4 + (size_t)2 * K * c.S3 * n * 4 + (size_t)c.D * n * 2;
 }
 
+uint16_t *relin32_planes(void *scratch, int n, int K, const Relin32Consts &c, long count) {
+    return (uint16_t *)((char *)scratch + (size_t)count * ((size_t)c.D * c.S3 * n * 4 + (size_t)2 * K * c.S3 * n * 4));
+}
+
 cudaError_t relin32_run(const DeviceParams *dP, int logn, int K, const Relin32 &r, const uint64_t *in3, uint64_t *out, long count,
                         void *scratch, cudaStream_t stream) {
     if (count <= 0) return cudaSuccess;
diff --git a/crcnn_b200/csrc/relin32.cuh b/crcnn_b200/csrc/relin32.cuh
--- a/crcnn_b200/csrc/relin32.cuh
+++ b/crcnn_b200/csrc/relin32.cuh
@@ -41,6 +41,8 @@
 
 size_t relin32_scratch_bytes(int n, int K, const Relin32Consts &c);
 
+uint16_t *relin32_planes(void *scratch, int n, int K, const Relin32Consts &c, long count);
+
 cudaError_t relin32_run(const DeviceParams *dP, int logn, int K, const Relin32 &r, const uint64_t *in3, uint64_t *out, long count,
                         void *scratch, cudaStream_t stream);
 
```

Measured after the change: 41.29 (median of 6 runs). About the same (+0.8%).
